# maplant/mgf

Hardware: AMD Instinct MI355X
Metric: contact_constraint_iters_per_sec (higher is better)
Workload: dtype f32

## Files before the change

mgf_amd/csrc/host_boundary.inc:

```

extern "C" mgf_status mgf_constraints_new(mgf_world* w, const mgf_body_ref* refs_a, const mgf_body_ref* refs_b, const mgf_manifold* manifolds,
                                          int64_t n, float dt, mgf_constraint* out, int64_t cap, int64_t* count) {
  if (!w || n < 0 || (n && (!refs_a || !refs_b || !manifolds))) return fail(MGF_ERR_INVALID, "bad argument");
  MGF_TRY(ctx_bind(w->ctx));
  MGF_TRY(perm_host(w));
  const uint32_t* so = w->permuted ? w->h_slot_of.data() : nullptr;
  std::vector<ManifoldRow> rows;
  std::vector<uint2> names;
  for (int64_t i = 0; i < n; ++i) {
    const mgf_body_ref& ra = refs_a[i];
    const mgf_body_ref& rb = refs_b[i];
    const mgf_manifold& m = manifolds[i];
    if (ra.tag != 0) return fail(MGF_ERR_STATIC_REF, "obj_a must be RigidBodyRef::Dynamic");
    if (ra.index >= w->n_owned) return fail(MGF_ERR_INVALID, "obj_a out of range");
    if (rb.tag == 0 && rb.index >= w->n_owned) return fail(MGF_ERR_INVALID, "obj_b out of range");
    if (rb.tag != 0 && rb.tag != 1) return fail(MGF_ERR_INVALID, "obj_b: unknown RigidBodyRef tag");
    if (rb.tag == 0 && rb.index == ra.index) return fail(MGF_ERR_INVALID, "a constraint needs two different bodies");
    if (m.n_contacts < 0 || m.n_contacts > MGF_MANIFOLD_CAP) return fail(MGF_ERR_INVALID, "manifold: n_contacts out of range");
    for (int32_t k = 0; k < m.n_contacts; ++k) {
      ManifoldRow r;
      r.a = ra.index; r.b = rb.tag == 0 ? rb.index : kNone;
      names.push_back(make_uint2(r.a, r.b));
      if (so) { r.a = so[r.a]; if (r.b != kNone) r.b = so[r.b]; }
      r.cb[0] = rb.center.x; r.cb[1] = rb.center.y; r.cb[2] = rb.center.z; r.fric_b = rb.friction;
// ... 53 lines not shown
  if (count) *count = (int64_t)s->cons.size();
  if (!out) return MGF_OK;
  if ((int64_t)s->cons.size() > cap) return fail(MGF_ERR_CAPACITY, "constraint buffer too small");
  if (!s->cons.empty()) memcpy(out, s->cons.data(), s->cons.size() * sizeof(mgf_constraint));
  return MGF_OK;
}
extern "C" mgf_status mgf_solver_solve(mgf_solver* s, mgf_world* w, int32_t iters, mgf_step_stats* stats) {
  if (!s || !w) return fail(MGF_ERR_INVALID, "NULL argument");
  if (iters < 0) return fail(MGF_ERR_INVALID, "iters must be >= 0");
  w->n = w->n_owned;
  mgf_status st = mgf_world_set_constraints(w, s->cons.data(), (int64_t)s->cons.size());
  if (st == MGF_OK) st = mgf_world_solve(w, iters, stats);
  if (st == MGF_OK && !s->cons.empty()) st = mgf_world_read_constraints(w, s->cons.data(), (int64_t)s->cons.size(), nullptr);
  return st;
}

template <class T>
static mgf_status clone_buf(mgf_ctx* ctx, DBuf<T>& dst, const DBuf<T>& src, size_t count) {
  if (count == 0 || !src.p) return MGF_OK;
  MGF_TRY(dst.ensure(count, ctx->stream));
  MGF_HIP_TRY(hipMemcpyAsync(dst.p, src.p, count * sizeof(T), hipMemcpyDeviceToDevice, ctx->stream));
  return MGF_OK;
}
extern "C" mgf_status mgf_world_clone(mgf_world* src, mgf_world** out) {
  if (!src || !out) return fail(MGF_ERR_INVALID, "NULL argument");
  *out = nullptr;
  mgf_world* w = nullptr;
  MGF_TRY(mgf_world_new(src->ctx, &src->params, &w));
  std::unique_ptr<mgf_world, void (*)(mgf_world*)> guard(w, mgf_world_free);
  mgf_ctx* ctx = src->ctx;
  const size_t n = src->n_owned;
  MGF_TRY(clone_buf(ctx, w->x, src->x, n)); MGF_TRY(clone_buf(ctx, w->q, src->q, n)); MGF_TRY(clone_buf(ctx, w->srec, src->srec, 4 * n));
  MGF_TRY(clone_buf(ctx, w->sp0, src->sp0, n)); MGF_TRY(clone_buf(ctx, w->sp1, src->sp1, n)); MGF_TRY(clone_buf(ctx, w->ctor, src->ctor, n));
  MGF_TRY(clone_buf(ctx, w->imb, src->imb, 3 * n)); MGF_TRY(clone_buf(ctx, w->delta, src->delta, n)); MGF_TRY(clone_buf(ctx, w->einfo, src->einfo, n));
  MGF_TRY(clone_buf(ctx, w->col0, src->col0, n)); MGF_TRY(clone_buf(ctx, w->col1, src->col1, n)); MGF_TRY(clone_buf(ctx, w->tb_c, src->tb_c, n));
  MGF_TRY(clone_buf(ctx, w->tb_r, src->tb_r, n)); MGF_TRY(clone_buf(ctx, w->fb_c, src->fb_c, n)); MGF_TRY(clone_buf(ctx, w->fb_r, src->fb_r, n));
  if (src->has_compound) {
    MGF_TRY(clone_buf(ctx, w->pcount, src->pcount, n));
    MGF_TRY(clone_buf(ctx, w->lp0, src->lp0, kMaxParts * n)); MGF_TRY(clone_buf(ctx, w->lp1, src->lp1, kMaxParts * n));
    MGF_TRY(clone_buf(ctx, w->wp0, src->wp0, kMaxParts * n)); MGF_TRY(clone_buf(ctx, w->wp1, src->wp1, kMaxParts * n));
    MGF_TRY(clone_buf(ctx, w->xl0, src->xl0, src->x_used)); MGF_TRY(clone_buf(ctx, w->xl1, src->xl1, src->x_used));
    MGF_TRY(clone_buf(ctx, w->xw0, src->xw0, src->x_used)); MGF_TRY(clone_buf(ctx, w->xw1, src->xw1, src->x_used));
    w->x_used = src->x_used;
  }
  if (src->permuted) {
    MGF_TRY(clone_buf(ctx, w->ext_of, src->ext_of, n)); MGF_TRY(clone_buf(ctx, w->slot_of, src->slot_of, n));
    w->permuted = true;
  }
  w->opt_resort_every = src->opt_resort_every; w->ticks_since_resort = src->ticks_since_resort;
  MGF_HIP_TRY(hipStreamSynchronize(ctx->stream));
  w->n = w->n_owned = src->n_owned;
  w->has_sphere = src->has_sphere; w->has_capsule = src->has_capsule; w->has_compound = src->has_compound; w->max_parts = src->max_parts;
  w->stats.n_bodies = w->n_owned;
  if (src->terrain) MGF_TRY(mgf_world_set_terrain(w, src->terrain.get()));
  for (const auto& ob : src->obstacles) MGF_TRY(mgf_world_add_obstacle(w, ob.get()));
  w->opt_constraint_order = src->opt_constraint_order; w->demo_tree = src->demo_tree; w->demo_leaf = src->demo_leaf;
  w->opt_flow6_poll_prio = src->opt_flow6_poll_prio; w->opt_flow6_slot_blocks = src->opt_flow6_slot_blocks; w->opt_resort_partition = src->opt_resort_partition; w->opt_part_cell_x8 = src->opt_part_cell_x8;
  w->opt_flow6_poll_k = src->opt_flow6_poll_k; w->opt_flow6_spec = src->opt_flow6_spec; w->opt_flow6_spec_wl = src->opt_flow6_spec_wl; w->opt_flow6_test_cap = src->opt_flow6_test_cap; w->opt_flow_trace = src->opt_flow_trace; w->opt_debug_bvh = src->opt_debug_bvh;
  w->opt_flow6_fcap = src->opt_flow6_fcap; w->opt_flow6_const_lds = src->opt_flow6_const_lds; w->opt_flow6_nimp_lds = src->opt_flow6_nimp_lds; w->opt_flow6_rec_lds = src->opt_flow6_rec_lds; w->opt_flow6_slot_margin = src->opt_flow6_slot_margin; w->opt_flow6_quad = src->opt_flow6_quad; w->opt_flow6_quad_max = src->opt_flow6_quad_max; w->opt_flow6_foreign_lds = src->opt_flow6_foreign_lds; w->opt_flow6_poll_waves = src->opt_flow6_poll_waves;
  w->opt_solver_mode = src->opt_solver_mode; w->opt_two_pass = src->opt_two_pass; w->opt_broadphase_tree = src->opt_broadphase_tree;
  w->opt_terrain_tree = src->opt_terrain_tree; w->opt_no_fused_narrowphase = src->opt_no_fused_narrowphase;
  w->opt_no_fused_scene_bounds = src->opt_no_fused_scene_bounds; w->opt_no_fused_terrain_rows = src->opt_no_fused_terrain_rows;
  w->opt_pair_brick = src->opt_pair_brick; w->opt_body_pack = src->opt_body_pack; w->opt_grid_min_frac_pct = src->opt_grid_min_frac_pct;
  w->grid_occupancy = src->grid_occupancy;
  w->opt_cell_fill = src->opt_cell_fill; w->opt_cell_fill_set = src->opt_cell_fill_set; w->opt_pipeline = src->opt_pipeline; w->opt_spin_wait = src->opt_spin_wait; w->opt_readback_kernel = src->opt_readback_kernel;
  w->opt_stream_ordered = src->opt_stream_ordered; w->opt_flow_blocks_per_cu = src->opt_flow_blocks_per_cu; w->opt_flow_sleep = src->opt_flow_sleep;
  w->opt_flow5_slow_x2 = src->opt_flow5_slow_x2; w->opt_flow5_poller = src->opt_flow5_poller; w->opt_flow5_block = src->opt_flow5_block;
  w->opt_flow5_test_cap = src->opt_flow5_test_cap; w->opt_time_solver_kernels = src->opt_time_solver_kernels; w->opt_phase_timing = src->opt_phase_timing;
  w->row_cap_t = src->row_cap_t; w->rev_cap = src->rev_cap; w->pair_brick_off = src->pair_brick_off; w->pair_brick_backoff = src->pair_brick_backoff; w->terrain_grid_off = src->terrain_grid_off; w->grid_too_wide = src->grid_too_wide;
  w->cap_t = src->cap_t; w->cap_p = src->cap_p; w->cap_c = src->cap_c; w->flow5_last_max = src->flow5_last_max;
  w->f6_fail_slots = src->f6_fail_slots; w->f6_fail_foreign = src->f6_fail_foreign; w->f6_fail_C = src->f6_fail_C; w->prev_C = src->prev_C;
  w->f6_last_slots = src->f6_last_slots; w->f6_last_foreign = src->f6_last_foreign; w->f6_last_msgs = src->f6_last_msgs;
  w->f6_last_block_msgs = src->f6_last_block_msgs; w->f6_prep_iters = src->f6_prep_iters;
  w->opt_merged_lists = src->opt_merged_lists; w->opt_fused_contacts = src->opt_fused_contacts; w->opt_front_rows = src->opt_front_rows; w->opt_front_rows_check = src->opt_front_rows_check; w->opt_side_stream = src->opt_side_stream; w->opt_wide_list = src->opt_wide_list; w->wide_engaged = src->wide_engaged; w->wide_hold = src->wide_hold;
  for (int k = 0; k < 3; ++k) { w->wide_ref[k] = src->wide_ref[k]; w->wide_limit[k] = src->wide_limit[k]; w->shape_rmax[k] = src->shape_rmax[k]; } w->front_rows_off = src->front_rows_off; w->opt_flow_max_blocks = src->opt_flow_max_blocks; w->opt_cells_in_integrate = src->opt_cells_in_integrate; w->opt_resort_every = src->opt_resort_every;
  for (int k = 0; k < 3; ++k) { w->h_scene_ext[k] = src->h_scene_ext[k]; w->h_scene_rmax[k] = src->h_scene_rmax[k]; }
  *out = guard.release();
  return MGF_OK;
}
```

mgf_amd/csrc/host_tick.inc:

```
enum TerrainPlan { kTerrainNone, kTerrainRows, kTerrainGrid };
static TerrainPlan terrain_plan(const mgf_world* w, bool two_pass) {
  if (two_pass || !w->terrain || w->terrain->m.tree.empty() || !w->n_owned) return kTerrainNone;
  return (w->terrain->grid.ready && !w->terrain_grid_off && !w->opt_terrain_tree && w->obstacles.empty()) ? kTerrainGrid : kTerrainRows;
}
static mgf_status world_integrate(mgf_world* w, float dt, bool complete, bool integrate, bool with_bounds, bool with_terrain_rows = false) {
  mgf_ctx* ctx = w->ctx;
  w->invalidate_tick_caches();
  if (w->n_owned == 0) return MGF_OK;
  SceneBounds* sb = with_bounds ? w->sb.p : nullptr;
  const uint32_t* guard = with_bounds ? w->scalars.p + 14 : nullptr;
  int* sb_part = (with_terrain_rows && integrate && with_bounds && !w->opt_no_fused_scene_bounds) ? w->sb_part.p : nullptr;
  w->bounds_cover = sb_part ? w->n_owned : 0u;
  MGF_TRY(w->bpk.ensure(4 * (size_t)std::max(w->n, w->n_owned), ctx->stream));
  w->pack_cover = integrate ? w->n_owned : 0u;
  CellSort cs;
  memset(&cs, 0, sizeof(cs));
  if (sb_part && w->plan.zero_launched && w->plan.n == w->n_owned && w->sbg_valid && w->opt_cells_in_integrate) {
    cs.grid = w->sb_grid.p; cs.shift = kMortonBits - 2 * (int)w->plan.levels; cs.min_frac = (float)w->opt_grid_min_frac_pct * 0.01f;
    cs.cell_of = w->cell_of.p; cs.rank = w->cell_rank.p; cs.cell_cnt = w->cell_cnt.p;
    w->cells_cover = w->n_owned; w->cells_levels = w->plan.levels;
  }
  WideSpec wd;
  memset(&wd, 0, sizeof(wd));
  w->wide_tick_on = false;
  if (sb_part && integrate && w->opt_wide_list && w->wide_engaged && w->wide_limit[0] > 0.0f) {
    MGF_TRY(w->wide_list.ensure(2 * (size_t)kWideCap, ctx->stream));
    for (int k = 0; k < 3; ++k) wd.limit[k] = w->wide_limit[k];
    wd.list = w->wide_list.p; wd.count = &w->sb.p->pad; wd.ext = w->ext_ptr();
    w->wide_tick_on = true;
  }
  if (with_terrain_rows && integrate && terrain_plan(w, w->opt_two_pass != 0) == kTerrainRows && !w->opt_no_fused_terrain_rows) {
    MGF_TRY(w->rows_t.ensure((size_t)w->n_owned * w->row_cap_t, ctx->stream));
    MGF_TRY(w->t_cnt.ensure((size_t)w->n_owned + 1, ctx->stream));
    MGF_TRY(w->near_list.ensure(3 * (size_t)w->n_owned, ctx->stream)); MGF_TRY(w->cs_sums.ensure(3 * kCsSumStride, ctx->stream));
    TerrainRowsTail tail{w->terrain->dev(w->d_err()), w->row_cap_t, w->rows_t.p, w->t_cnt.p, w->d_err() + 1, w->opt_fused_contacts ? w->near_list.p : nullptr, w->cs_sums.p + 2 * kCsSumStride};
    k_integrate<<<nblk(w->n_owned), kBlock, 0, ctx->stream>>>(w->bodies(), w->n_owned, dt, w->params.fat_margin, complete ? 1 : 0, 1, sb, guard, tail, sb_part, cs, wd);
    w->terrain_rows_done = true;
  } else {
    k_integrate<<<nblk(w->n_owned), kBlock, 0, ctx->stream>>>(w->bodies(), w->n_owned, dt, w->params.fat_margin, complete ? 1 : 0, integrate ? 1 : 0,
                                                        sb, guard, NoTail(), sb_part, cs, wd);
  }
  LAUNCH_CHECK();
  return MGF_OK;
}
extern "C" mgf_status mgf_world_complete_motion(mgf_world* w) {
  if (!w) return fail(MGF_ERR_INVALID, "world is NULL");
  MGF_TRY(ctx_bind(w->ctx));
  MGF_TRY(world_integrate(w, 0.0f, true, false, false));
  MGF_HIP_TRY(hipStreamSynchronize(w->ctx->stream));
  return MGF_OK;
}
extern "C" mgf_status mgf_world_integrate(mgf_world* w, float dt) {
  if (!w) return fail(MGF_ERR_INVALID, "world is NULL");
  MGF_TRY(ctx_bind(w->ctx));
  MGF_TRY(world_integrate(w, dt, false, true, false));
  MGF_HIP_TRY(hipStreamSynchronize(w->ctx->stream));
  return MGF_OK;
}

static mgf_status launch_pairs(mgf_world* w, int ka, int kb, const uint32_t* work, const uint32_t* m_ptr, uint32_t cap, bool pack_ok) {
  if (cap == 0) return MGF_OK;
  hipStream_t s = w->ctx->stream;
  Bodies B = w->bodies();
  if (!pack_ok) B.bpk = nullptr;
  unsigned g = nblk(cap);
  if (ka == 0 && kb == 0) k_narrow_pairs<0, 0><<<g, kBlock, 0, s>>>(B, work, m_ptr, w->p_owner.p, w->p_cand.p, w->p_nc.p, w->p_out.p);
  else if (ka == 0 && kb == 1) k_narrow_pairs<0, 1><<<g, kBlock, 0, s>>>(B, work, m_ptr, w->p_owner.p, w->p_cand.p, w->p_nc.p, w->p_out.p);
  else if (ka == 1 && kb == 0) k_narrow_pairs<1, 0><<<g, kBlock, 0, s>>>(B, work, m_ptr, w->p_owner.p, w->p_cand.p, w->p_nc.p, w->p_out.p);
  else k_narrow_pairs<1, 1><<<g, kBlock, 0, s>>>(B, work, m_ptr, w->p_owner.p, w->p_cand.p, w->p_nc.p, w->p_out.p);
  LAUNCH_CHECK();
  return MGF_OK;
}
static mgf_status launch_terrain(mgf_world* w, int ka, const TerrainDev& M, const uint32_t* work, const uint32_t* m_ptr, uint32_t cap, bool pack_ok) {
  if (cap == 0) return MGF_OK;
  hipStream_t s = w->ctx->stream;
  Bodies B = w->bodies();
  if (!pack_ok) B.bpk = nullptr;
  unsigned g = nblk(cap);
  if (ka == 0) k_narrow_terrain<0><<<g, kBlock, 0, s>>>(B, M, work, m_ptr, w->t_owner.p, w->t_cand.p, w->t_nc.p, w->t_out.p);
  else k_narrow_terrain<1><<<g, kBlock, 0, s>>>(B, M, work, m_ptr, w->t_owner.p, w->t_cand.p, w->t_nc.p, w->t_out.p);
  LAUNCH_CHECK();
  return MGF_OK;
}

static mgf_status links_ensure(mgf_world* w, uint32_t cap_c, bool zero = false) {
  hipStream_t s = w->ctx->stream;
  uint32_t n = w->n;
  MGF_TRY(w->c_ab.ensure(std::max(cap_c, 1u), s)); MGF_TRY(w->c_succ.ensure(std::max(cap_c, 1u), s)); MGF_TRY(w->c_pred.ensure(2 * (size_t)std::max(cap_c, 1u), s));
  MGF_TRY(w->deg.ensure(n + 1, s)); MGF_TRY(w->adj_off.ensure(n + 1, s)); MGF_TRY(w->adj_fill.ensure(n + 1, s));
  MGF_TRY(w->adj_list.ensure(2 * (size_t)std::max(cap_c, 1u), s));
  if (zero) {
    MGF_HIP_TRY(hipMemsetAsync(w->deg.p, 0, (n + 1) * 4, s));
    MGF_HIP_TRY(hipMemsetAsync(w->adj_fill.p, 0, (n + 1) * 4, s));
  }
  return MGF_OK;
}
static mgf_status build_dag(mgf_world* w, uint32_t cap_c) {
  mgf_ctx* ctx = w->ctx;
  hipStream_t s = ctx->stream;
  uint32_t n = w->n;
  w->depth = 0;
  if (cap_c == 0) return MGF_OK;
  if (cap_c >= kSuccId) return fail(MGF_ERR_CAPACITY, "too many constraints");
  MGF_TRY(prim_exclusive_scan_u32(ctx, w->deg.p, w->adj_off.p, (size_t)n + 1));
  k_adj_fill<<<nblk(cap_c), kBlock, 0, s>>>(w->c_ab.p, &w->sc.p->C, w->adj_off.p, w->adj_fill.p, w->adj_list.p);
  LAUNCH_CHECK();
  k_chain<<<nblk(n), kBlock, 0, s>>>(n, w->links(), w->adj_off.p, w->adj_list.p);
  LAUNCH_CHECK();
  return MGF_OK;
}
// ... 170 lines not shown
      bool ok = false;
      MGF_TRY(flow6_plan(w, cap_c, w->f6_prep_iters ? w->f6_prep_iters : 10u, &ok));
      if (ok) { flow6_zero_entries(w, cap_c, z, 8); w->flow6_zeroed = true; }
    }
    if (solver_follows && w->opt_solver_mode == 5) {
      bool ok = false;
      MGF_TRY(flow5_plan(w, cap_c, &ok));
      if (ok) { flow5_zero_entries(w, cap_c, z, 8); w->flow5_zeroed = true; }
    }
    if (early) {
      k_tick_clear<<<256, kBlock, 0, s>>>(z, w->sb.p, w->d_err(), w->scalars.p + 14, &w->sc.p->fail, speculative ? 1 : 0, w->sb_part.p);
      w->plan.zero_launched = true;
    } else {
      if (bounds_done) { z.sb = w->sb.p; z.sb_part = w->sb_part.p; }
      k_zero_many<<<256, kBlock, 0, s>>>(z);
      w->plan.zero_launched = false;
    }
    LAUNCH_CHECK();
  }
  return MGF_OK;
}
static mgf_status collide_enqueue(mgf_world* w, float dt, bool solver_follows = false) {
  mgf_ctx* ctx = w->ctx;
  hipStream_t s = ctx->stream;
  const uint32_t n = w->n;
  StepCounts* sc = w->sc.p;
  if (n == 0) { MGF_HIP_TRY(hipMemsetAsync(sc, 0, sizeof(StepCounts), s)); return MGF_OK; }
  Bodies B = w->bodies();
  const float min_frac = (float)w->opt_grid_min_frac_pct * 0.01f;
  const bool cleared = w->plan.zero_launched && w->plan.n == n && w->plan.cap_c == w->cap_c && w->plan.solver_follows == solver_follows && w->cap_p != 0;
  w->plan.zero_launched = false;
  const bool bounds_done = w->bounds_cover == n && n > 0;
  const bool rows_done = w->terrain_rows_done;
  const bool pack_ok = w->pack_cover == n && n > 0 && w->opt_body_pack;
  if (!cleared) MGF_TRY(collide_prepare(w, solver_follows, false, false));
  const uint32_t cap_t = w->cap_t, cap_p = w->cap_p, cap_c = w->cap_c;
  const uint32_t levels = w->plan.levels, cells = w->plan.cells, nblocks = cells / kBlock;
  if (!pack_ok) B.bpk = nullptr;
  const bool cells_done = cleared && bounds_done && w->cells_cover == n && w->cells_levels == w->plan.levels;
  w->invalidate_tick_caches();
  const bool fold_in_morton = cleared && bounds_done;
  if (!bounds_done) {
    k_scene_bounds<<<std::min<unsigned>(nblk(n), 64u), kBlock, 0, s>>>(w->fb_c.p, w->fb_r.p, n, w->sb.p);
    LAUNCH_CHECK();
  }
  if (!cells_done) {
    k_morton_count<<<nblk(n), kBlock, 0, s>>>(w->fb_c.p, n, w->sb.p, kMortonBits - 2 * (int)levels, w->cell_of.p, w->cell_rank.p, w->cell_cnt.p, min_frac, make_uint3(0, 0, 0),
                                              fold_in_morton ? w->sb_part.p : nullptr, w->sb.p);
    LAUNCH_CHECK();
  }
  const SceneBounds* grid_box_of = cells_done ? w->sb_grid.p : nullptr;
  MGF_TRY(tick_scan(w, 0, w->cell_cnt.p, w->cell_lo.p, nullptr, nullptr, (size_t)cells + 1, nullptr, nullptr, cells_done ? w->sb_part.p : nullptr));
  Lbvh T;
  T.nodes = w->lnodes.p; T.leaves = w->leaves.p; T.sidx = w->sidx.p; T.cell_lo = w->cell_lo.p;
  T.n = n; T.levels = levels; T.err = w->d_err();
  T.dbg = nullptr;
  T.ext = w->ext_ptr();
  const bool two_pass = (w->opt_two_pass != 0 || w->tick_two_pass) && !w->demo_rows_ready;
  const bool use_grid = !two_pass && !w->opt_broadphase_tree && !w->grid_too_wide;
  const bool demo = w->demo_rows_ready;
  const bool fused = use_grid && !w->has_capsule && !w->has_compound && !w->opt_no_fused_narrowphase && !demo;
  T.lcol = nullptr; T.ltb = nullptr;
  if (fused) { MGF_TRY(w->lcol.ensure(2 * (size_t)n, s)); T.lcol = w->lcol.p; }
  const bool wide_now = w->wide_tick_on && bounds_done && use_grid && !two_pass && !demo;
  const float3 wlim = wide_now ? make_float3(w->wide_limit[0], w->wide_limit[1], w->wide_limit[2]) : make_float3(0.0f, 0.0f, 0.0f);
  const bool brick = use_grid && !demo && w->opt_pair_brick && w->pair_brick_off == 0 && !wide_now;
  if (w->pair_brick_off) --w->pair_brick_off;
  w->ts->brick = brick;
  if (use_grid && !demo) { MGF_TRY(w->ltb.ensure(2 * (size_t)n, s)); T.ltb = w->ltb.p; }
  if (brick) {
    if (!w->pair_brick_attr) {
// ... 43 lines not shown
    }
    MGF_TRY(w->near_ids.ensure(w->n_owned, s)); MGF_TRY(w->tpos.ensure(n + 1, s));
    const FaceGrid FG = w->terrain->face_grid();
    k_near_list<<<nblk(w->n_owned), kBlock, 0, ts>>>(w->tb_c.p, w->tb_r.p, w->n_owned, M, FG.sb, 1e-3f, w->near_ids.p, w->cs_sums.p + 2 * kCsSumStride, w->scalars.p + 14);
    LAUNCH_CHECK();
    TerrainNear A;
    A.M = M; A.G = FG; A.near_ids = w->near_ids.p; A.near_cnt = w->cs_sums.p + 2 * kCsSumStride; A.face_of_rank = w->terrain->grid.face_of_rank.p;
    const uint32_t region_cap = slot_space / kTnRegions;
    A.pad_abs = 1e-3f; A.cap_t = cap_t; A.cnt = w->front_cnt.p; A.region_cap = region_cap; A.slot_body = w->t_owner.p; A.slot_rank = w->t_cand.p; A.tpos = w->tpos.p; A.t_cnt = w->t_cnt.p;
    A.overflow = w->d_err() + 1; A.too_wide = w->d_err() + 5; A.guard = w->scalars.p + 14;
    A.check = w->opt_front_rows_check ? 1u : 0u;
#ifndef MGF_TN_LANES
#define MGF_TN_LANES 16
#endif
    constexpr int kTnLanes = MGF_TN_LANES;
    const unsigned tgb = 8u * std::max(1u, std::min((unsigned)((w->n_owned + (kBlock / kTnLanes) - 1) / (kBlock / kTnLanes) + 7u) / 8u, 256u));
    k_terrain_near<kTnLanes><<<tgb, kBlock, 0, ts>>>(B, A);
    LAUNCH_CHECK();
    TerrainTests X;
    X.M = M; X.face_of_rank = w->terrain->grid.face_of_rank.p; X.slot_body = w->t_owner.p; X.slot_rank = w->t_cand.p; X.cnt = w->front_cnt.p; X.region_cap = region_cap;
    X.t_out = w->t_out.p; X.tcn = w->tcn.p; X.sum_ct = w->cs_sums.p + kCsSumStride; X.flag = w->d_err() + 8; X.overflow = w->d_err() + 1;
    k_terrain_tests<<<nblk((size_t)region_cap * kTnRegions), kBlock, 0, ts>>>(B, X);
    LAUNCH_CHECK();
    if (forked) MGF_HIP_TRY(hipEventRecord(w->ts->ev_join, ctx->aux));
  }
  if (tc_job) {
    const uint32_t t_stride0 = w->has_compound ? 2u * (w->max_parts > 2u ? (uint32_t)kMaxParts : 2u) : 2u;
    MGF_TRY(w->t_out.ensure((size_t)t_stride0 * cap_t, s)); MGF_TRY(w->tpos.ensure(n + 1, s));
    TerrainContacts A;
    A.M = M; A.near_list = w->near_list.p; A.near_cnt = w->cs_sums.p + 2 * kCsSumStride;
    A.n_faces = (uint32_t)(w->terrain->faces.size() / 3); A.n_verts = (uint32_t)w->terrain->verts.size(); A.cap_row_t = w->row_cap_t; A.cap_t = cap_t;
    A.rows_t = w->rows_t.p; A.sums = w->cs_sums.p; A.t_out = w->t_out.p; A.tcn = w->tcn.p; A.tpos = w->tpos.p; A.guard = w->scalars.p + 14;
    A.check = (front_rows && w->opt_front_rows_check) ? 1u : 0u; A.flag = w->d_err() + 8;
    A.col1 = w->col1.p; A.pcount = w->has_compound ? w->pcount.p : nullptr; A.wp0 = w->wp0.p; A.wp1 = w->wp1.p;
    const unsigned tg = std::max(1u, std::min(nblk((size_t)w->n_owned * kTcLanes / 8 + 1), 256u));
    if (front_rows) {
      hipStream_t ts = s;
      if (w->opt_side_stream && !w->opt_phase_timing) {
        if (!ctx->aux) {
          int lo = 0, hi = 0;
          MGF_HIP_TRY(hipDeviceGetStreamPriorityRange(&lo, &hi));
          MGF_HIP_TRY(hipStreamCreateWithPriority(&ctx->aux, hipStreamNonBlocking, w->opt_side_stream >= 2 ? lo : hi));
        }
        if (!w->ts->ev_fork) { MGF_HIP_TRY(hipEventCreateWithFlags(&w->ts->ev_fork, hipEventDisableTiming)); MGF_HIP_TRY(hipEventCreateWithFlags(&w->ts->ev_join, hipEventDisableTiming)); }
        MGF_HIP_TRY(hipEventRecord(w->ts->ev_fork, s));
        MGF_HIP_TRY(hipStreamWaitEvent(ctx->aux, w->ts->ev_fork, 0));
        ts = ctx->aux; forked = true;
      }
      if (w->has_compound) k_terrain_contacts<2><<<tg, kBlock, 0, ts>>>(A);
      else k_terrain_contacts<1><<<tg, kBlock, 0, ts>>>(A);
      LAUNCH_CHECK();
      if (forked) MGF_HIP_TRY(hipEventRecord(w->ts->ev_join, ts));
      k_scatter_leaves<<<nblk(n), kBlock, 0, s>>>(T, w->fb_c.p, w->fb_r.p, w->cell_of.p, w->cell_rank.p, w->brank.p, w->col0.p, w->delta.p, w->tb_c.p, w->tb_r.p, w->sb.p, 1e-3f, min_frac, grid_box_of, wlim, w->n_owned);
    } else if (w->opt_fused_contacts >= 2) {
      k_terrain_contacts<0><<<tg, kBlock, 0, s>>>(A);
      LAUNCH_CHECK();
      k_scatter_leaves<<<nblk(n), kBlock, 0, s>>>(T, w->fb_c.p, w->fb_r.p, w->cell_of.p, w->cell_rank.p, w->brank.p, w->col0.p, w->delta.p, w->tb_c.p, w->tb_r.p, w->sb.p, 1e-3f, min_frac, grid_box_of, wlim, w->n_owned);
    } else {
      k_scatter_leaves_tc<0><<<nblk(n) + tg, kBlock, 0, s>>>(T, w->fb_c.p, w->fb_r.p, w->cell_of.p, w->cell_rank.p, w->brank.p, w->col0.p, w->delta.p, w->tb_c.p, w->tb_r.p, w->sb.p, 1e-3f, min_frac, A, tg, grid_box_of, wlim, w->n_owned);
    }
  } else {
    k_scatter_leaves<<<nblk(n), kBlock, 0, s>>>(T, w->fb_c.p, w->fb_r.p, w->cell_of.p, w->cell_rank.p, w->brank.p, w->col0.p, w->delta.p, w->tb_c.p, w->tb_r.p, w->sb.p, 1e-3f, min_frac, grid_box_of, wlim, w->n_owned);
  }
  LAUNCH_CHECK();
  w->sidx_valid = n == w->n_owned;
  if (!use_grid) {
    k_lbvh_low<<<nblocks, kBlock, 0, s>>>(T, w->sub_lo.p, w->sub_hi.p);
    LAUNCH_CHECK();
    if (levels > 4) { k_lbvh_top<<<1, 1024, 0, s>>>(T, w->sub_lo.p, w->sub_hi.p, w->sub2_lo.p, w->sub2_hi.p); LAUNCH_CHECK(); }
  }
  MGF_TRY(phase_mark(w, 1, s));
  MGF_TRY(w->t_cand.ensure(cap_t, s)); MGF_TRY(w->t_owner.ensure(cap_t, s));
  MGF_TRY(w->p_cand.ensure(cap_p, s)); MGF_TRY(w->p_owner.ensure(cap_p, s));
  MGF_TRY(w->t_nc.ensure(cap_t, s)); MGF_TRY(w->p_nc.ensure(cap_p, s));
  MGF_TRY(w->t_pre.ensure(cap_t, s)); MGF_TRY(w->p_pre.ensure(cap_p, s));
  const uint32_t MP = w->max_parts > 2u ? (uint32_t)kMaxParts : 2u;
  const bool big = w->max_parts > (uint32_t)kMaxParts;
  const uint32_t t_stride = w->has_compound ? 2u * (big ? w->max_parts : MP) : 2u, p_stride = w->has_compound ? MP * MP : 1u;
  static_assert(kBigKeep == (uint32_t)(kMaxParts * kMaxParts), "k_narrow_pairs_big writes k_narrow_pairs_parts<kMaxParts>'s records");
  MGF_TRY(w->t_out.ensure((size_t)t_stride * cap_t, s)); MGF_TRY(w->p_out.ensure((size_t)p_stride * cap_p, s));
  if (!two_pass) {
    MGF_TRY(w->rows.ensure((size_t)n * kRowCap, s));
    MGF_TRY(w->rows_t.ensure((size_t)n * w->row_cap_t, s, rows_done, (size_t)w->n_owned * w->row_cap_t));
    if (front_rows && terrain_any && terrain_grid) {
    } else if (M.n_nodes && w->n_owned && !rows_done) {
      if (terrain_grid) {
        const uint32_t per_block = kCoopBlock / kCoopLanes;
        const uint32_t tg = 8 * (((w->n_owned + per_block - 1) / per_block + 7) / 8);
        k_terrain_grid<<<tg, kCoopBlock, 0, s>>>(B, w->n_owned, nullptr, M, w->terrain->face_grid(), 1e-3f, w->row_cap_t, w->rows_t.p, w->t_cnt.p,
                                                 w->d_err() + 1, w->d_err() + 5);
      } else {
        k_terrain_rows<<<nblk(w->n_owned), kBlock, 0, s>>>(B, w->n_owned, M, w->row_cap_t, w->rows_t.p, w->t_cnt.p, w->d_err() + 1);
      }
      LAUNCH_CHECK();
    }
// ... 78 lines not shown
  } else if (two_pass) {
    k_candidates<true><<<8 * xcd_blocks_per(n), kBlock, 0, s>>>(B, n, w->n_owned, T, M, 1e-3f, nullptr, nullptr, w->t_off.p, w->p_off.p, w->t_cand.p, w->t_owner.p,
                                                  w->p_cand.p, w->p_owner.p, sc);
    if (n_obs && w->n_owned) {
      LAUNCH_CHECK();
      k_obstacle_candidates<true><<<nblk(w->n_owned), kBlock, 0, s>>>(B, w->n_owned, w->d_obs.p, n_obs, w->t_cnt.p, w->t_off.p, w->t_cand.p, w->t_owner.p, sc);
    }
  } else {
    k_rows_to_csr<<<nblk(n), kBlock, 0, s>>>(sc, n, w->row_cap_t, terrain_grid ? w->terrain->grid.face_of_rank.p : nullptr, w->rows_t.p, w->rows.p, w->t_off.p, w->p_off.p, w->t_cand.p, w->t_owner.p, w->p_cand.p, w->p_owner.p);
  }
  LAUNCH_CHECK();
  MGF_TRY(phase_mark(w, 2, s));
  bool mixed = w->has_sphere && w->has_capsule;
  if (lists_merged || front_rows) {
  } else if (w->has_compound) {
    if (cap_p && big) {
      k_narrow_pairs_big<<<std::min(std::max(cap_p / 4u, 1u), 4096u), kBlock, 0, s>>>(B, &sc->Mp, w->p_owner.p, w->p_cand.p, w->p_nc.p, w->p_out.p, w->scalars.p + 24);
      LAUNCH_CHECK();
    } else if (cap_p) {
      if (MP == 2u) k_narrow_pairs_parts<2><<<nblk(cap_p), kBlock, 0, s>>>(B, &sc->Mp, w->p_owner.p, w->p_cand.p, w->p_nc.p, w->p_out.p);
      else k_narrow_pairs_parts<kMaxParts><<<nblk(cap_p), kBlock, 0, s>>>(B, &sc->Mp, w->p_owner.p, w->p_cand.p, w->p_nc.p, w->p_out.p);
      LAUNCH_CHECK();
    }
    if ((M.n_nodes || n_obs) && cap_t && big) {
      k_narrow_terrain_big<<<std::min(std::max(cap_t / 4u, 1u), 4096u), kBlock, 0, s>>>(B, M, &sc->Mt, w->t_owner.p, w->t_cand.p, w->t_nc.p, w->t_out.p, t_stride);
      LAUNCH_CHECK();
    } else if ((M.n_nodes || n_obs) && cap_t) {
      if (MP == 2u) k_narrow_terrain_parts<2><<<nblk(cap_t), kBlock, 0, s>>>(B, M, &sc->Mt, w->t_owner.p, w->t_cand.p, w->t_nc.p, w->t_out.p);
      else k_narrow_terrain_parts<kMaxParts><<<nblk(cap_t), kBlock, 0, s>>>(B, M, &sc->Mt, w->t_owner.p, w->t_cand.p, w->t_nc.p, w->t_out.p);
      LAUNCH_CHECK();
    }
  } else if (!mixed) {
    int k = w->has_capsule ? 1 : 0;
    if (!fused) MGF_TRY(launch_pairs(w, k, k, nullptr, &sc->Mp, cap_p, pack_ok));
    if (M.n_nodes || n_obs) MGF_TRY(launch_terrain(w, k, M, nullptr, &sc->Mt, cap_t, pack_ok));
  } else {
    MGF_TRY(w->work_lists.ensure(4 * (size_t)cap_p + 2 * (size_t)cap_t, s));
    uint32_t* lists_p = w->work_lists.p;
    uint32_t* lists_t = w->work_lists.p + 4 * (size_t)cap_p;
    k_bin_pairs<<<nblk(cap_p), kBlock, 0, s>>>(B, &sc->Mp, cap_p, w->p_owner.p, w->p_cand.p, lists_p, sc->bins);
    LAUNCH_CHECK();
    for (int ty = 0; ty < 4; ++ty) MGF_TRY(launch_pairs(w, ty >> 1, ty & 1, lists_p + (size_t)ty * cap_p, &sc->bins[ty], cap_p, pack_ok));
    if (M.n_nodes || n_obs) {
      k_bin_terrain<<<nblk(cap_t), kBlock, 0, s>>>(B, &sc->Mt, cap_t, w->t_owner.p, lists_t, sc->bins + 4);
      LAUNCH_CHECK();
      for (int ty = 0; ty < 2; ++ty) MGF_TRY(launch_terrain(w, ty, M, lists_t + (size_t)ty * cap_t, &sc->bins[4 + ty], cap_t, pack_ok));
    }
  }
  if (n_obs && cap_t) {
    k_narrow_obstacles<<<nblk(cap_t), kBlock, 0, s>>>(B, w->d_obs.p, &sc->Mt, w->t_owner.p, w->t_cand.p, w->t_nc.p, w->t_out.p, t_stride);
    LAUNCH_CHECK();
  }
  MGF_TRY(phase_mark(w, 3, s));
  MGF_TRY(w->cnt.ensure(n + 1, s)); MGF_TRY(w->base.ensure(n + 1, s)); MGF_TRY(w->tcn.ensure(n + 1, s));
  if (!contacts_fused && !front_rows) {
  if (!lists_merged) {
    k_count_contacts<<<nblk(n), kBlock, 0, s>>>(sc, n, w->t_off.p, w->p_off.p, w->t_nc.p, fused ? nullptr : w->p_nc.p, w->p_cand.p, w->t_pre.p, w->p_pre.p, w->cnt.p,
                                                demo ? 1 : 0, w->tcn.p, w->ext_ptr());
    LAUNCH_CHECK();
  }
  {
    ScanEpilogue E;
    memset(&E, 0, sizeof(E));
    E.kind = 2; E.cap_a = cap_c; E.sc = sc;
    MGF_TRY(tick_scan(w, 2, w->cnt.p, w->base.p, nullptr, nullptr, (size_t)n + 1, &E));
  }
  TerrainSetup TS;
  memset(&TS, 0, sizeof(TS));
  if (M.n_nodes || n_obs) {
    TS.M = M; TS.t_owner = w->t_owner.p; TS.t_nc = w->t_nc.p; TS.t_pre = w->t_pre.p; TS.t_in = w->t_out.p; TS.in_stride = t_stride; TS.blocks = nblk(cap_t);
    if (n_obs) { TS.t_cand = w->t_cand.p; TS.obs_center = w->d_obs_center.p; }
  }
  if (fused) k_setup_pairs<true><<<TS.blocks + nblk(cap_p), kBlock, 0, s>>>(B, sc, w->p_owner.p, w->p_cand.p, nullptr, w->p_pre.p, nullptr, w->base.p, dt,
                                                                            w->params.baumgarte, w->params.penetration_slop, w->cons_nat.p, w->c_ab.p, w->degb.p, w->rev.p,
                                                                            w->rev_cap, w->d_err() + 7, p_stride, w->d_err() + 8, TS, w->ext_ptr());
  else k_setup_pairs<false><<<TS.blocks + nblk(cap_p), kBlock, 0, s>>>(B, sc, w->p_owner.p, w->p_cand.p, w->p_nc.p, w->p_pre.p, w->p_out.p, w->base.p, dt,
                                                                       w->params.baumgarte, w->params.penetration_slop, w->cons_nat.p, w->c_ab.p, w->degb.p, w->rev.p,
                                                                       w->rev_cap, w->d_err() + 7, p_stride, w->d_err() + 8, TS, w->ext_ptr());
  LAUNCH_CHECK();
// ... 214 lines not shown
```

mgf_amd/csrc/host_tiles.inc:

```
template <class Batch, class Tile>
static mgf_status tile_batches(hipStream_t s, void (*kern)(Batch), const Tile* tiles, const uint32_t* blocks, int L) {
  for (int i0 = 0; i0 < L; i0 += kTileBatch) {
    Batch A;
    memset(&A, 0, sizeof(A));
    const int cnt = std::min(kTileBatch, L - i0);
    uint32_t mx = 0;
    for (int k = 0; k < cnt; ++k) { A.t[k] = tiles[i0 + k]; mx = std::max(mx, blocks[i0 + k]); }
    if (!mx) continue;
    kern<<<dim3(mx, (unsigned)cnt), kBlock, 0, s>>>(A);
    LAUNCH_CHECK();
  }
  return MGF_OK;
}
static mgf_status select_describe(mgf_world* w, float x_left, float x_right, float x_lo, float x_hi, uint32_t* ids_l, uint32_t* ids_r, uint32_t* ids_m, SelTile* S) {
  const uint32_t n = w->n_owned, nb = nblk(n);
  MGF_TRY(w->sel_blk.ensure(4 * (size_t)nb + 4, w->ctx->stream));
  S->fb_c = w->fb_c.p; S->fb_r = w->fb_r.p; S->x = w->x.p; S->n = n;
  S->x_left = x_left; S->x_right = x_right; S->x_lo = x_lo; S->x_hi = x_hi;
  S->blk = w->sel_blk.p; S->tot = w->sel_blk.p + 4 * (size_t)nb; S->tot_host = nullptr;
  S->ids_l = ids_l; S->ids_r = ids_r; S->ids_m = ids_m;
  return MGF_OK;
}
static mgf_status select_counts(hipStream_t s, const SelTile* sel, int L) {
  std::vector<uint32_t> blocks((size_t)L);
// ... 46 lines not shown
  MGF_TRY(grow_keep(w, w->pcount, 1, need));
  MGF_TRY(grow_keep(w, w->lp0, kMaxParts, need)); MGF_TRY(grow_keep(w, w->lp1, kMaxParts, need));
  MGF_TRY(grow_keep(w, w->wp0, kMaxParts, need)); MGF_TRY(grow_keep(w, w->wp1, kMaxParts, need));
  return MGF_OK;
}
static mgf_status raise_parts_for_records(mgf_world* w, const float* rec, int64_t m, uint32_t stride_floats, uint32_t at) {
  if (m <= 0 || !rec) return MGF_OK;
  MGF_TRY(w->mig_cnt.ensure(2, w->ctx->stream));
  MGF_HIP_TRY(hipMemsetAsync(w->mig_cnt.p, 0, 8, w->ctx->stream));
  k_record_max_parts<<<nblk(m), kBlock, 0, w->ctx->stream>>>(rec, (uint32_t)m, stride_floats, at, w->mig_cnt.p);
  LAUNCH_CHECK();
  uint32_t pc = 0;
  MGF_TRY(d2h(w->ctx, &pc, w->mig_cnt.p, 1));
  if (pc > (uint32_t)kTileParts) return fail(MGF_ERR_INVALID, "a record claims more parts than a tile record carries");
  if (pc > 2u && w->max_parts <= 2u) return mgf_world_set_option(w, "body_kinds", 12);
  if (pc > 0u && !w->has_compound) return mgf_world_set_option(w, "body_kinds", 4);
  return MGF_OK;
}
static mgf_status world_import_ghosts2(mgf_world* w, const float* src, int64_t n_ghost, const float* src2, int64_t n_first);
extern "C" mgf_status mgf_world_import_ghosts(mgf_world* w, const float* src, int64_t n_ghost) {
  if (w && src && n_ghost > 0 && !w->opt_stream_ordered) { MGF_TRY(ctx_bind(w->ctx)); MGF_TRY(raise_parts_for_records(w, src, n_ghost, (uint32_t)kGhostFloats, 36u)); }
  return world_import_ghosts2(w, src, n_ghost, nullptr, n_ghost);
}
static mgf_status world_import_ghosts_prepare(mgf_world* w, const float* src, int64_t n_ghost, const float* src2, int64_t n_first, ImpTile* I) {
  memset(I, 0, sizeof(*I));
  if (w) w->sbg_valid = false;
  if (!w || (n_ghost && !src && !src2) || n_ghost < 0 || n_first < 0 || (n_first < n_ghost && !src2) || (n_first > 0 && n_ghost > 0 && !src)) return fail(MGF_ERR_INVALID, "bad argument");
  MGF_TRY(ctx_bind(w->ctx));
  MGF_TRY(world_identity(w));
  size_t need = (size_t)w->n_owned + (size_t)n_ghost;
  if (need > 0x7FFFFFF0ull) return fail(MGF_ERR_INVALID, "too many bodies");
  MGF_TRY(grow_keep(w, w->x, 1, need)); MGF_TRY(grow_keep(w, w->q, 1, need)); MGF_TRY(grow_keep(w, w->srec, 4, need));
  MGF_TRY(grow_keep(w, w->sp0, 1, need)); MGF_TRY(grow_keep(w, w->sp1, 1, need)); MGF_TRY(grow_keep(w, w->ctor, 1, need));
  MGF_TRY(grow_keep(w, w->imb, 3, need)); MGF_TRY(grow_keep(w, w->delta, 1, need)); MGF_TRY(grow_keep(w, w->einfo, 1, need));
  MGF_TRY(grow_keep(w, w->col0, 1, need)); MGF_TRY(grow_keep(w, w->col1, 1, need)); MGF_TRY(grow_keep(w, w->tb_c, 1, need));
  MGF_TRY(grow_keep(w, w->tb_r, 1, need)); MGF_TRY(grow_keep(w, w->fb_c, 1, need)); MGF_TRY(grow_keep(w, w->fb_r, 1, need));
  MGF_TRY(grow_parts(w, need));
  MGF_TRY(grow_keep(w, w->bpk, 4, need));
  w->pack_cover = (w->pack_cover >= w->n_owned && w->n_owned > 0) ? (uint32_t)need : 0u;
  if (n_ghost > 0) {
    const bool join = w->bounds_cover == w->n_owned && w->n == w->n_owned && w->n_owned > 0;
    I->B = w->bodies(); I->n_owned = w->n_owned; I->m = (uint32_t)n_ghost; I->m1 = (uint32_t)std::min<int64_t>(n_first, n_ghost);
    I->fat_margin = w->params.fat_margin; I->in = src; I->in2 = src2; I->sb_part = join ? w->sb_part.p : nullptr;
    I->rec1 = I->rec2 = (uint32_t)kGhostFloats;
    w->bounds_cover = join ? (uint32_t)need : 0u;
  } else if (w->n != w->n_owned) {
    w->bounds_cover = 0;
  }
  w->n = (uint32_t)need;
  w->constraints_ready = false;
  return MGF_OK;
}
static mgf_status world_import_ghosts2(mgf_world* w, const float* src, int64_t n_ghost, const float* src2, int64_t n_first) {
  ImpTile I;
  MGF_TRY(world_import_ghosts_prepare(w, src, n_ghost, src2, n_first, &I));
  const uint32_t blocks = nblk(I.m);
  MGF_TRY((tile_batches<ImpBatch, ImpTile>(w->ctx->stream, k_import_ghosts, &I, &blocks, 1)));
  return sync_unless_ordered(w);
}
extern "C" mgf_status mgf_world_select_tile(mgf_world* w, float x_left, float x_right, float x_lo, float x_hi, uint32_t* ids_left,
                                            uint32_t* ids_right, uint32_t* ids_migrants, int64_t cap, int64_t* counts) {
  if (!w || !counts) return fail(MGF_ERR_INVALID, "NULL argument");
  MGF_TRY(ctx_bind(w->ctx));
  MGF_TRY(world_identity(w));
  mgf_ctx* ctx = w->ctx;
  hipStream_t s = ctx->stream;
  counts[0] = counts[1] = counts[2] = counts[3] = 0;
  if (w->n_owned == 0) return MGF_OK;
  SelTile S;
  MGF_TRY(select_describe(w, x_left, x_right, x_lo, x_hi, ids_left, ids_right, ids_migrants, &S));
  MGF_TRY(select_counts(s, &S, 1));
// ... 59 lines not shown
  if (!trusted) {
    uint32_t* pin = static_cast<uint32_t*>(ctx->pinned);
    MGF_HIP_TRY(hipMemcpyAsync(pin, w->mig_cnt.p, 4, hipMemcpyDeviceToHost, s));
    MGF_HIP_TRY(hipStreamSynchronize(s));
    if (pin[0]) return fail(MGF_ERR_INVALID, "remove_bodies: an id is out of range or listed twice");
  }
  const uint32_t n_new = n - (uint32_t)n_ids;
  if (n_new) {
    k_compact_put<<<dim3(nblk(n_new), row_words), kBlock, 0, s>>>(w->bodies(), n, n_new, w->bscan_l.p, w->mig_tmp.p);
    LAUNCH_CHECK();
  }
  w->n_owned = w->n = n_new;
  w->stats.n_bodies = n_new;
  w->sidx_valid = false;
  w->demo_tree.clear(); w->demo_leaf.clear();
  return sync_unless_ordered(w);
}
extern "C" mgf_status mgf_world_remove_bodies(mgf_world* w, const uint32_t* ids, int64_t n_ids) { return remove_bodies_impl(w, ids, n_ids, false); }
static mgf_status import_migrants_impl(mgf_world* w, const float* src, int64_t n_in, uint32_t kinds_hint, const float* src2 = nullptr, int64_t n_first = -1) {
  if (n_first < 0 || n_first > n_in) n_first = n_in;
  if (!w || n_in < 0 || (n_first > 0 && !src) || (n_first < n_in && (!src2 || !kinds_hint))) return fail(MGF_ERR_INVALID, "bad argument");
  w->invalidate_tick_caches();
  MGF_TRY(ctx_bind(w->ctx));
  MGF_TRY(world_identity(w));
  w->n = w->n_owned;
  w->constraints_ready = false;
  if (n_in == 0) return MGF_OK;
  size_t need = (size_t)w->n_owned + (size_t)n_in;
  if (need > 0x7FFFFFF0ull) return fail(MGF_ERR_INVALID, "too many bodies");
  w->sbg_valid = false; w->ptrs_out = false;
  if (!kinds_hint) MGF_TRY(raise_parts_for_records(w, src, n_in, 4u * (uint32_t)kMigrantWords, 4u * 20u));
  MGF_TRY(grow_keep(w, w->x, 1, need)); MGF_TRY(grow_keep(w, w->q, 1, need)); MGF_TRY(grow_keep(w, w->srec, 4, need));
  MGF_TRY(grow_keep(w, w->sp0, 1, need)); MGF_TRY(grow_keep(w, w->sp1, 1, need)); MGF_TRY(grow_keep(w, w->ctor, 1, need));
  MGF_TRY(grow_keep(w, w->imb, 3, need)); MGF_TRY(grow_keep(w, w->delta, 1, need)); MGF_TRY(grow_keep(w, w->einfo, 1, need));
  MGF_TRY(grow_keep(w, w->col0, 1, need)); MGF_TRY(grow_keep(w, w->col1, 1, need)); MGF_TRY(grow_keep(w, w->tb_c, 1, need));
  MGF_TRY(grow_keep(w, w->tb_r, 1, need)); MGF_TRY(grow_keep(w, w->fb_c, 1, need)); MGF_TRY(grow_keep(w, w->fb_r, 1, need));
  MGF_TRY(grow_parts(w, need));
  k_import_migrants<<<nblk((size_t)n_in * kMigrantWords), kBlock, 0, w->ctx->stream>>>(w->bodies(), w->n_owned, (uint32_t)n_in,
                                                                                      reinterpret_cast<const float4*>(src), kTileParts,
                                                                                      reinterpret_cast<const float4*>(src2), (uint32_t)n_first);
  LAUNCH_CHECK();
  w->n_owned = w->n = (uint32_t)need;
  w->stats.n_bodies = w->n_owned;
  w->sidx_valid = false;
  if (kinds_hint) {
    if (kinds_hint & 1u) w->has_sphere = true;
    if (kinds_hint & 2u) w->has_capsule = true;
    return MGF_OK;
  }
  MGF_TRY(w->mig_cnt.ensure(2, w->ctx->stream));
  MGF_HIP_TRY(hipMemsetAsync(w->mig_cnt.p, 0, 8, w->ctx->stream));
  k_kind_mask<<<nblk(n_in), kBlock, 0, w->ctx->stream>>>(w->col1.p, w->has_compound ? w->pcount.p : nullptr, w->n_owned - (uint32_t)n_in, (uint32_t)n_in, w->mig_cnt.p);
  LAUNCH_CHECK();
  uint32_t mask = 0;
  MGF_TRY(d2h(w->ctx, &mask, w->mig_cnt.p, 1));
  if (mask & 1) w->has_sphere = true;
  if (mask & 2) w->has_capsule = true;
  return MGF_OK;
}
extern "C" mgf_status mgf_world_import_migrants(mgf_world* w, const float* src, int64_t n_in) { return import_migrants_impl(w, src, n_in, 0u); }
extern "C" mgf_status mgf_world_set_tags(mgf_world* w, const uint32_t* tags, int64_t n) {
  if (!w || (n && !tags)) return fail(MGF_ERR_INVALID, "NULL argument");
  if ((uint64_t)n != (uint64_t)w->n_owned) return fail(MGF_ERR_INVALID, "one tag per owned body");
  MGF_TRY(ctx_bind(w->ctx));
  if (n == 0) return MGF_OK;
  MGF_TRY(w->bflag_l.ensure((size_t)n + 1, w->ctx->stream));
  if (w->permuted) {
    MGF_TRY(perm_host(w));
    std::vector<uint32_t> t((size_t)n);
    for (size_t i = 0; i < (size_t)n; ++i) t[w->h_slot_of[i]] = tags[i];
    MGF_TRY(h2d(w->ctx, w->bflag_l.p, t.data(), (size_t)n));
  } else {
    MGF_TRY(h2d(w->ctx, w->bflag_l.p, tags, (size_t)n));
  }
  k_tags_set<<<nblk(n), kBlock, 0, w->ctx->stream>>>(w->ctor.p, w->bflag_l.p, (uint32_t)n);
  LAUNCH_CHECK();
  MGF_HIP_TRY(hipStreamSynchronize(w->ctx->stream));
  return MGF_OK;
}
extern "C" mgf_status mgf_world_read_tags(mgf_world* w, uint32_t* tags, int64_t cap) {
  if (!w || (cap && !tags)) return fail(MGF_ERR_INVALID, "NULL argument");
  if ((uint64_t)cap < (uint64_t)w->n_owned) return fail(MGF_ERR_CAPACITY, "tag buffer too small");
  MGF_TRY(ctx_bind(w->ctx));
  const uint32_t n = w->n_owned;
  if (n == 0) return MGF_OK;
// ... 43 lines not shown
```

mgf_amd/csrc/host_world.inc:

```
struct mgf_world {
  mgf_ctx* ctx = nullptr;
  mgf_params params;
  uint32_t n = 0;
  uint32_t n_owned = 0;
  bool has_sphere = false, has_capsule = false;
  bool has_compound = false;
  uint32_t max_parts = 0;
  DBuf<uint32_t> pcount;
  DBuf<float4> xl0, xl1, xw0, xw1;
  uint32_t x_used = 0;
  DBuf<float4> lp0, lp1, wp0, wp1;
  DBuf<uint32_t> bflag_l, bscan_l;
  DBuf<uint32_t> sel_blk;
  DBuf<uint32_t> mig_cnt;
  DBuf<float4> mig_tmp;
  DBuf<float> state_pack;
  void* state_pin = nullptr; size_t state_pin_bytes = 0;
  DBuf<float4> x, q, srec, sp0, sp1, ctor, imb, delta, einfo, col0, col1, tb_c, tb_r, fb_c, fb_r;
  DBuf<float4> bpk;
  DBuf<uint32_t> ext_of, ext_new, slot_of;
  DBuf<float4> perm_tmp;
  bool permuted = false;
  bool sidx_valid = false;
  int64_t opt_resort_every = -1;
  uint64_t ticks_since_resort = 0, n_resorts = 0;
  std::vector<uint32_t> h_ext_of, h_slot_of;
  bool h_perm_valid = false;
  const uint32_t* ext_ptr() const { return permuted ? ext_of.p : nullptr; }
  DBuf<uint32_t> part_keys[2], part_vals[2];
  int64_t opt_part_cell_x8 = 4;
  int64_t opt_resort_partition = 1;
  float h_scene_ext[3] = {0, 0, 0};
  float h_scene_rmax[3] = {0, 0, 0};
  bool list_generic = false;
  DBuf<uint32_t> f6_cslot, f6_clist;
  DBuf<uint32_t> iota;
  size_t iota_n = 0;
  int64_t opt_flow6_slot_blocks = 1;
  DBuf<uint32_t> cnt_e, base_e, canon;
  bool canon_ready = false;
  std::unique_ptr<mgf_mesh> terrain;
  std::vector<std::unique_ptr<mgf_compound>> obstacles;
  DBuf<CompoundDev> d_obs;
  DBuf<float4> d_obs_center;
  DBuf<uint32_t> cell_of, cell_rank, sidx;
  DBuf<QNode> lnodes;
  DBuf<LeafRec> leaves;
  DBuf<float4> ltb;
  DBuf<float4> lcol;
  int64_t opt_no_fused_narrowphase = 0;
  int64_t opt_grid_min_frac_pct = 50;
  int64_t opt_merged_lists = 1;
  int64_t opt_cells_in_integrate = 1;
  int64_t opt_front_rows = 1;
  int64_t opt_wide_list = 1;
  bool wide_engaged = false, wide_tick_on = false;
  float wide_ref[3] = {0, 0, 0}, wide_limit[3] = {0, 0, 0};
  float shape_rmax[3] = {0, 0, 0};
  uint32_t wide_hold = 0, wide_last = 0;
  uint64_t n_wide_ticks = 0, n_wide_overflows = 0;
  uint64_t n_path_ticks[4] = {0, 0, 0, 0};
  DBuf<float4> wide_list;
  DBuf<float4> q_bc, q_br;
  DBuf<uint32_t> q_cnt, q_start, q_items, q_large, q_misc, q_off, q_vals;
  DBuf<ParticleIn> q_parts; DBuf<int32_t> q_ign, q_hits; DBuf<float> q_boxes;
  DBuf<MovingIn> q_casts;
  uint32_t q_last_large = 0, q_last_cells = 0;
  float q_last_build_ms = 0.0f, q_last_run_ms = 0.0f;
  int64_t opt_side_stream = 1;
  int64_t opt_front_rows_check = 0;
  bool front_rows_off = false;
  int64_t opt_fused_contacts = 1;
  int64_t opt_body_pack = 1;
  int64_t opt_pair_brick = 1;
  uint64_t pair_brick_slow = 0;
  uint32_t pair_brick_off = 0;
  uint32_t pair_brick_backoff = 256;
  bool pair_brick_attr = false;
  DBuf<float4> sub_lo, sub_hi, sub2_lo, sub2_hi;
  DBuf<uint32_t> cell_lo, cell_cnt;
  DBuf<uint32_t> t_cnt, p_cnt, t_off, p_off, t_cand, t_owner, p_cand, p_owner, rows, rows_t;
  int64_t opt_solver_mode = 6;
  DBuf<uint32_t> flow_arr, flow_arr5;
  DBuf<uint64_t> flow_trace;
  DBuf<uint32_t> brank, f5_shared, f5_gcnt, f5_lslot, f5_wg_cnt;
  DBuf<F5Row> f5_table;
  bool flow5_zeroed = false;
  bool f6_fail_known = false;
  uint32_t f6_fail_host = 0;
  bool f6_standby = false;
  uint32_t f6_edges_block = 0;
  bool links_ready = false;
  bool flow5_ok = false, flow5_prepped = false;
  uint32_t f5_nb = 0, f5_nblocks = 0;
  DBuf<uint4> f6_binfo;
  DBuf<uint32_t> f6_bref, f6_fcnt, f6_fbody, f6_nslots, f6_in_key, f6_in_cnt, f6_out_key, f6_out_val, f6_chan_prefix;
  DBuf<uint8_t> f6_cflags, f6_skipwb;
  DBuf<F6Row> f6_table;
  DBuf<uint4> f6_mbox;
  DBuf<unsigned long long> f6_tails;
  uint32_t f6_mbox_cap = 0;
  uint32_t f6_epoch = 0;
  uint32_t f6_fcap = 512, f6_slot_cap = 0, f6_rows = 0;
  uint32_t f6_last_slots = 0, f6_last_foreign = 0;
  uint32_t f6_fail_slots = 0, f6_fail_foreign = 0, f6_fail_C = 0, prev_C = 0;
  uint64_t n_flow6_skipped = 0;
// ... 102 lines not shown
  View<SceneBounds> sb;
  uint32_t Mt = 0, Mp = 0, C = 0, Ct = 0, depth = 0, last_launches = 0, lvl_cap = 0;
  size_t order_cap_iters = 0;
  bool constraints_ready = false;
  float last_dt = 0.0f;
  float last_rmax_x = 0.0f;
  float grid_occupancy = 1.0f;
  int64_t opt_time_solver_kernels = 0;
  int64_t opt_phase_timing = 0;
  struct TickSlot {
    hipEvent_t ev[8] = {};
    uint32_t ev_set = 0;
    std::vector<hipEvent_t> kev;
    size_t kev_used = 0;
    bool brick = false;
    bool fused = false;
    bool front_rows = false;
    bool contacts_fused = false;
    bool cells_early = false;
    hipEvent_t ev_fork = nullptr, ev_join = nullptr;
    uint32_t* pin = nullptr;
    uint32_t* pin_dev = nullptr;
    uint32_t seq = 0;
  };
  static constexpr uint32_t kPinWords = 4096, kPinSeqWord = 4095;
  void* pin_block = nullptr;
  TickSlot slots[2];
  TickSlot* ts = &slots[0];
  mgf_step_stats stats;

  Bodies bodies() {
    Bodies B;
    B.x = x.p; B.q = q.p; B.srec = srec.p; B.sp0 = sp0.p; B.sp1 = sp1.p; B.ctor = ctor.p; B.imb = imb.p; B.bpk = bpk.p; B.delta = delta.p;
    B.einfo = einfo.p; B.col0 = col0.p; B.col1 = col1.p; B.tb_c = tb_c.p; B.tb_r = tb_r.p; B.fb_c = fb_c.p; B.fb_r = fb_r.p;
    B.pcount = has_compound ? pcount.p : nullptr; B.lp0 = lp0.p; B.lp1 = lp1.p; B.wp0 = wp0.p; B.wp1 = wp1.p;
    B.xl0 = xl0.p; B.xl1 = xl1.p; B.xw0 = xw0.p; B.xw1 = xw1.p;
    return B;
  }
  uint32_t* d_cnt() { return scalars.p; }
  uint32_t* d_err() { return scalars.p + 3; }
  uint32_t flow5_narrow_cap() const { return f5_narrow_cap(f5_nb); }
  Flow5 flow5() {
    Flow5 F;
    F.sidx = sidx.p; F.brank = brank.p; F.shared = reinterpret_cast<uint8_t*>(f5_shared.p);
    F.gcnt = f5_gcnt.p; F.arr5 = flow_arr5.p; F.lslot = f5_lslot.p; F.wg_cnt = f5_wg_cnt.p;
    F.table = f5_table.p;
    F.fail = d_err() + 4; F.max_block = d_err() + 6;
    F.cap_fast = flow5_wide ? kF5MaxFast : flow5_narrow_cap(); F.cap_slow = flow5_wide ? kF5MaxSlow : flow5_narrow_cap();
    F.cap_all = flow5_wide ? kF5MaxCons : flow5_narrow_cap();
    if (opt_flow5_test_cap > 0) F.cap_all = std::min<uint32_t>(F.cap_all, (uint32_t)opt_flow5_test_cap);
    F.slow_x2 = (uint32_t)opt_flow5_slow_x2;
    F.poller = opt_flow5_poller < 0 ? (flow5_wide ? 0u : 1u) : (uint32_t)opt_flow5_poller;
    F.nb = f5_nb; F.nblocks = f5_nblocks; F.n = n;
    return F;
  }
  ConsLinks links() { ConsLinks K; K.ab = c_ab.p; K.succ = c_succ.p; K.pred = c_pred.p; return K; }
  Frontier frontier() { Frontier F; F.order = order.p; F.lvl_off = lvl_off.p; F.cnt = d_cnt(); return F; }
};
static mgf_status phase_mark(mgf_world* w, int k, hipStream_t s) {
  if (!w->opt_phase_timing) return MGF_OK;
  MGF_HIP_TRY(hipEventRecord(w->ts->ev[k], s));
  w->ts->ev_set |= 1u << k;
  return MGF_OK;
}
static mgf_status phase_ms(mgf_world* w, int a, int b, float* ms) {
  *ms = 0.0f;
  if (!w->opt_phase_timing || (w->ts->ev_set & (1u << a)) == 0u || (w->ts->ev_set & (1u << b)) == 0u) return MGF_OK;
// ... 75 lines not shown
  if (!strcmp(key, "flow6_nimp_lds")) { w->opt_flow6_nimp_lds = value; return MGF_OK; }
  if (!strcmp(key, "flow6_rec_lds")) { w->opt_flow6_rec_lds = value; return MGF_OK; }
  if (!strcmp(key, "flow6_slot_margin")) { if (value < 0 || value > 1024) return fail(MGF_ERR_INVALID, "flow6_slot_margin: 0..1024"); w->opt_flow6_slot_margin = value; return MGF_OK; }
  if (!strcmp(key, "flow6_quad")) { w->opt_flow6_quad = value; return MGF_OK; }
  if (!strcmp(key, "flow6_quad_max")) { if (value < -1 || value > 1000000) return fail(MGF_ERR_INVALID, "flow6_quad_max out of range"); w->opt_flow6_quad_max = value; return MGF_OK; }
  if (!strcmp(key, "flow6_foreign_lds")) { w->opt_flow6_foreign_lds = value; return MGF_OK; }
  if (!strcmp(key, "flow6_test_cap")) { w->opt_flow6_test_cap = value; return MGF_OK; }
  if (!strcmp(key, "flow6_poll_prio")) { if (value < 0 || value > 3) return fail(MGF_ERR_INVALID, "flow6_poll_prio: 0..3"); w->opt_flow6_poll_prio = value; return MGF_OK; }
  if (!strcmp(key, "flow6_spec_wl")) { if (value < -1 || value > 8) return fail(MGF_ERR_INVALID, "flow6_spec_wl: -1..8"); w->opt_flow6_spec_wl = value; return MGF_OK; }
  if (!strcmp(key, "flow6_spec")) { if (value < 0 || value > 8) return fail(MGF_ERR_INVALID, "flow6_spec: 0 (by the launch), 1..8"); w->opt_flow6_spec = value; return MGF_OK; }
  if (!strcmp(key, "flow6_poll_waves")) { if (value < 0 || value > 4) return fail(MGF_ERR_INVALID, "flow6_poll_waves out of range"); w->opt_flow6_poll_waves = value; return MGF_OK; }
  if (!strcmp(key, "flow6_poll_k")) { if (value < 1 || value > 4) return fail(MGF_ERR_INVALID, "flow6_poll_k out of range"); w->opt_flow6_poll_k = value; return MGF_OK; }
  if (!strcmp(key, "flow_blocks_per_cu")) { w->opt_flow_blocks_per_cu = value; w->flow_grid = 0; w->flowk_grid = 0; return MGF_OK; }
  if (!strcmp(key, "flow_sleep")) { w->opt_flow_sleep = value; return MGF_OK; }
  if (!strcmp(key, "flow5_poller")) { w->opt_flow5_poller = value < 0 ? -1 : (value ? 1 : 0); return MGF_OK; }
  if (!strcmp(key, "flow5_slow_x2")) { if (value < 1 || value > 16) return fail(MGF_ERR_INVALID, "flow5_slow_x2 out of range"); w->opt_flow5_slow_x2 = value; return MGF_OK; }
  if (!strcmp(key, "flow5_test_cap")) { w->opt_flow5_test_cap = value; return MGF_OK; }
  if (!strcmp(key, "flow5_block")) { w->opt_flow5_block = value; w->flow5_prepped = false; return MGF_OK; }
  if (!strcmp(key, "no_fused_narrowphase")) { w->opt_no_fused_narrowphase = value; return MGF_OK; }
  if (!strcmp(key, "pair_brick")) { w->opt_pair_brick = value; return MGF_OK; }
  if (!strcmp(key, "merged_lists")) { w->opt_merged_lists = value; return MGF_OK; }
  if (!strcmp(key, "fused_contacts")) { w->opt_fused_contacts = value; return MGF_OK; }
  if (!strcmp(key, "front_rows")) { w->opt_front_rows = value; return MGF_OK; }
  if (!strcmp(key, "side_stream")) { w->opt_side_stream = value; return MGF_OK; }
  if (!strcmp(key, "wide_list")) { w->opt_wide_list = value; if (!value) w->wide_engaged = false; return MGF_OK; }
  if (!strcmp(key, "front_rows_check")) { w->opt_front_rows_check = value; return MGF_OK; }
  if (!strcmp(key, "cells_in_integrate")) { w->opt_cells_in_integrate = value; return MGF_OK; }
  if (!strcmp(key, "flow_spin_limit")) { if (value < 0 || value > (4 << 20)) return fail(MGF_ERR_INVALID, "flow_spin_limit: 0 .. 4194304"); w->opt_flow_spin_limit = value; return MGF_OK; }
  if (!strcmp(key, "flow_max_blocks")) {
    if (value < 0 || value > 4096) return fail(MGF_ERR_INVALID, "flow_max_blocks: 0 (one workgroup per CU) .. 4096");
    w->opt_flow_max_blocks = value; w->flow_grid = 0; w->flowk_grid = 0; w->flow5_prepped = false; w->flow6_prepped = false;
    return MGF_OK;
  }
  if (!strcmp(key, "body_pack")) { w->opt_body_pack = value; return MGF_OK; }
  if (!strcmp(key, "grid_min_frac_pct")) { if (value < 0 || value > 100) return fail(MGF_ERR_INVALID, "grid_min_frac_pct: 0..100"); w->opt_grid_min_frac_pct = value; return MGF_OK; }
  if (!strcmp(key, "cell_fill")) { if (value < 1 || value > 1024) return fail(MGF_ERR_INVALID, "cell_fill out of range"); w->opt_cell_fill = value; w->opt_cell_fill_set = true; return MGF_OK; }
  if (!strcmp(key, "no_fused_scene_bounds")) { w->opt_no_fused_scene_bounds = value; return MGF_OK; }
  if (!strcmp(key, "no_fused_terrain_rows")) { w->opt_no_fused_terrain_rows = value; return MGF_OK; }
  if (!strcmp(key, "part_cell_x8")) { if (value < 0 || value > 64) return fail(MGF_ERR_INVALID, "part_cell_x8: 0..64"); w->opt_part_cell_x8 = value; return MGF_OK; }
  if (!strcmp(key, "resort_partition")) { w->opt_resort_partition = value; return MGF_OK; }
  if (!strcmp(key, "flow6_slot_blocks")) { w->opt_flow6_slot_blocks = value; return MGF_OK; }
  if (!strcmp(key, "resort_every")) {
    if (value < -1 || value > 1000000) return fail(MGF_ERR_INVALID, "resort_every out of range");
    w->opt_resort_every = value;
    if (value == 0) MGF_TRY(world_identity(w));
    return MGF_OK;
  }
  if (!strcmp(key, "pipeline")) { w->opt_pipeline = value; return MGF_OK; }
  if (!strcmp(key, "spin_wait")) { w->opt_spin_wait = value; return MGF_OK; }
  if (!strcmp(key, "readback_kernel")) { w->opt_readback_kernel = value != 0; return MGF_OK; }
  if (!strcmp(key, "stream_ordered")) { w->opt_stream_ordered = value; return MGF_OK; }
  if (!strcmp(key, "body_kinds")) {
    if (value & 1) w->has_sphere = true;
    if (value & 2) w->has_capsule = true;
    if ((value & 12) == 12) w->max_parts = std::max(w->max_parts, (uint32_t)kMaxParts);
    else if (value & 4) w->max_parts = std::max(w->max_parts, 2u);
    if ((value & 4) && !w->has_compound) {
      MGF_TRY(ctx_bind(w->ctx));
      const size_t o = w->n_owned;
      std::vector<uint32_t> pz(o, 0u);
      std::vector<float4> fz(kMaxParts * o, make_float4(0, 0, 0, 0));
      MGF_TRY(append(w->ctx, w->pcount, 0, pz));
      MGF_TRY(append(w->ctx, w->lp0, 0, fz)); MGF_TRY(append(w->ctx, w->lp1, 0, fz));
      MGF_TRY(append(w->ctx, w->wp0, 0, fz)); MGF_TRY(append(w->ctx, w->wp1, 0, fz));
      w->has_compound = true;
    }
    return MGF_OK;
// ... 199 lines not shown
      float best_len = 0.0f;
      for (int k = 0; k < 3; ++k) {
        const float len = (hi[k] - lo[k]) / (float)(1u << bits[k]);
        if (bits[k] < 10u && len * 0.5f >= 2.0f * rmax[k] && len * 0.5f > 0.0f && len > best_len) { best = k; best_len = len; }
      }
      if (best < 0) break;
      ++bits[best];
    }
    G.bits[0] = bits[0]; G.bits[1] = bits[1]; G.bits[2] = bits[2];
  }
  const uint32_t cells = 1u << (G.bits[0] + G.bits[1] + G.bits[2]);
  G.levels = levels; G.n_faces = (uint32_t)nf;
  MGF_TRY(G.fb_c.ensure(nf, s)); MGF_TRY(G.fb_r.ensure(nf, s)); MGF_TRY(G.cell_of.ensure(nf, s)); MGF_TRY(G.cell_rank.ensure(nf, s));
  MGF_TRY(G.cell_cnt.ensure((size_t)cells + 1, s)); MGF_TRY(G.cell_lo.ensure((size_t)cells + 1, s)); MGF_TRY(G.sidx.ensure(nf, s));
  MGF_TRY(G.brank.ensure(nf, s)); MGF_TRY(G.leaves.ensure(nf, s)); MGF_TRY(G.sb.ensure(1, s));
  MGF_TRY(G.rank_of_face.ensure(nf, s)); MGF_TRY(G.face_of_rank.ensure(nf, s)); MGF_TRY(G.leaf_of_face.ensure(nf, s));
  MGF_TRY(G.parent.ensure(std::max<size_t>(parent.size(), 1), s));
  MGF_TRY(h2d(ctx, G.fb_c.p, bc.data(), nf)); MGF_TRY(h2d(ctx, G.fb_r.p, br.data(), nf));
  MGF_TRY(h2d(ctx, G.rank_of_face.p, rank_of.data(), nf)); MGF_TRY(h2d(ctx, G.face_of_rank.p, face_of.data(), nf));
  MGF_TRY(h2d(ctx, G.leaf_of_face.p, leaf_of.data(), nf)); MGF_TRY(h2d(ctx, G.parent.p, parent.data(), parent.size()));
  MGF_HIP_TRY(hipMemsetAsync(G.cell_cnt.p, 0, ((size_t)cells + 1) * 4, s));
  SceneBounds sb0;
  for (int k = 0; k < 3; ++k) { sb0.lo[k] = 0x7FFFFFFF; sb0.hi[k] = (int)0x80000000; sb0.rmax[k] = 0; }
  sb0.n_refits = 0; sb0.pad = 0; sb0.pad2 = 0;
  MGF_TRY(h2d(ctx, G.sb.p, &sb0, 1));
  k_scene_bounds<<<std::min<unsigned>(nblk(nf), 256u), kBlock, 0, s>>>(G.fb_c.p, G.fb_r.p, (uint32_t)nf, G.sb.p);
  LAUNCH_CHECK();
  if (G.bits[0] + G.bits[1] + G.bits[2] == 0) return MGF_OK;
  k_morton_count<<<nblk(nf), kBlock, 0, s>>>(G.fb_c.p, (uint32_t)nf, G.sb.p, kMortonBits - 2 * (int)levels, G.cell_of.p, G.cell_rank.p, G.cell_cnt.p, 0.0f,
                                             make_uint3(G.bits[0], G.bits[1], G.bits[2]));
  LAUNCH_CHECK();
  MGF_TRY(prim_exclusive_scan_u32(ctx, G.cell_cnt.p, G.cell_lo.p, (size_t)cells + 1));
  FaceGrid FG = t->face_grid();
  k_scatter_leaves<<<nblk(nf), kBlock, 0, s>>>(FG.T, G.fb_c.p, G.fb_r.p, G.cell_of.p, G.cell_rank.p, G.brank.p, nullptr, nullptr, nullptr, nullptr, nullptr, 0.0f, 0.0f);
  LAUNCH_CHECK();
  MGF_HIP_TRY(hipStreamSynchronize(s));
  G.ready = true;
  return MGF_OK;
}

extern "C" mgf_status mgf_world_set_terrain(mgf_world* w, const mgf_mesh* mesh) {
  if (!w) return fail(MGF_ERR_INVALID, "world is NULL");
  w->invalidate_tick_caches();
  MGF_TRY(ctx_bind(w->ctx));
  if (!mesh) { w->terrain.reset(); return MGF_OK; }
  std::unique_ptr<mgf_mesh> t(new mgf_mesh());
  t->ctx = w->ctx;
  t->x = mesh->x;
  t->verts = mesh->verts;
  t->faces = mesh->faces;
  t->m.tree = mesh->m.tree;
  t->geom_version = 1;
  MGF_TRY(t->sync());
  MGF_TRY(build_face_grid(t.get()));
  w->terrain = std::move(t);
  w->terrain_grid_off = false;
  return MGF_OK;
}


extern "C" mgf_status mgf_world_add_obstacle(mgf_world* w, const mgf_compound* c) {
  if (!w || !c) return fail(MGF_ERR_INVALID, "NULL argument");
  if (w->obstacles.size() >= kObstacleMax) return fail(MGF_ERR_CAPACITY, "at most 256 obstacles");
  if (c->comps.size() >= kObstacleCompMax) return fail(MGF_ERR_CAPACITY, "an obstacle holds at most 2^18 components");
  MGF_TRY(ctx_bind(w->ctx));
  w->invalidate_tick_caches();
  std::unique_ptr<mgf_compound> o(new mgf_compound());
// ... 44 lines not shown
    Comp local = k; local.p = k.p + -px;
    M3 inv;
    if (!invert(tensor_of(local, mass[i]), &inv)) return fail(MGF_ERR_SINGULAR, "inertia tensor is not invertible (physics.rs:212)");
    float inv_mass = 1.0f / mass[i];
    V3 force = mk3(world_force[i].x, world_force[i].y, world_force[i].z) * mass[i];
    hx[i] = make_float4(px.x, px.y, px.z, 0.0f);
    hq[i] = make_float4(pq.s, pq.v.x, pq.v.y, pq.v.z);
    hs[4 * i] = make_float4(0, 0, 0, 0);
    hs[4 * i + 1] = make_float4(0, 0, inv_mass, inv.c[0].x);
    hs[4 * i + 2] = make_float4(inv.c[0].y, inv.c[0].z, inv.c[1].x, inv.c[1].y);
    hs[4 * i + 3] = make_float4(inv.c[1].z, inv.c[2].x, inv.c[2].y, inv.c[2].z);
    h0[i] = make_float4(force.x, force.y, force.z, restitution[i]);
    h1[i] = make_float4(0, 0, 0, friction[i]);
    uint32_t kind_bits = (uint32_t)k.kind;
    float kf; memcpy(&kf, &kind_bits, 4);
    hc[i] = make_float4(kf, k.r, half_h, 0.0f);
    for (int c = 0; c < 3; ++c) hi[3 * i + c] = make_float4(inv.c[c].x, inv.c[c].y, inv.c[c].z, 0.0f);
    hd[i] = make_float4(0, 0, 0, friction[i]);
    he[i] = make_float4(px.x, px.y, px.z, restitution[i]);
    c0[i] = make_float4(k.p.x, k.p.y, k.p.z, k.r);
    c1[i] = make_float4(k.d.x, k.d.y, k.d.z, kf);
    Box tb = swept_bounds(k, mk3(0, 0, 0));
    tc[i] = make_float4(tb.c.x, tb.c.y, tb.c.z, 0); tr[i] = make_float4(tb.r.x, tb.r.y, tb.r.z, 0);
    V3 fm = mk3(w->params.fat_margin, w->params.fat_margin, w->params.fat_margin);
    V3 frr = tb.r + fm;
    fc[i] = tc[i]; fr[i] = make_float4(frr.x, frr.y, frr.z, 0);
    w->shape_rmax[0] = std::max(w->shape_rmax[0], frr.x); w->shape_rmax[1] = std::max(w->shape_rmax[1], frr.y); w->shape_rmax[2] = std::max(w->shape_rmax[2], frr.z);
  }
  mgf_ctx* ctx = w->ctx;
  size_t o = w->n_owned;
  w->sbg_valid = false; w->ptrs_out = false;
  MGF_TRY(append(ctx, w->x, o, hx)); MGF_TRY(append(ctx, w->q, o, hq)); MGF_TRY(append(ctx, w->srec, 4 * o, hs));
  MGF_TRY(append(ctx, w->sp0, o, h0)); MGF_TRY(append(ctx, w->sp1, o, h1)); MGF_TRY(append(ctx, w->ctor, o, hc));
  MGF_TRY(append(ctx, w->imb, 3 * o, hi)); MGF_TRY(append(ctx, w->delta, o, hd)); MGF_TRY(append(ctx, w->einfo, o, he));
  MGF_TRY(append(ctx, w->col0, o, c0)); MGF_TRY(append(ctx, w->col1, o, c1)); MGF_TRY(append(ctx, w->tb_c, o, tc));
  MGF_TRY(append(ctx, w->tb_r, o, tr)); MGF_TRY(append(ctx, w->fb_c, o, fc)); MGF_TRY(append(ctx, w->fb_r, o, fr));
  if (w->has_compound) {
    std::vector<uint32_t> pz(N, 0u);
    std::vector<float4> fz(kMaxParts * N, make_float4(0, 0, 0, 0));
    MGF_TRY(append(ctx, w->pcount, o, pz));
    MGF_TRY(append(ctx, w->lp0, kMaxParts * o, fz)); MGF_TRY(append(ctx, w->lp1, kMaxParts * o, fz));
    MGF_TRY(append(ctx, w->wp0, kMaxParts * o, fz)); MGF_TRY(append(ctx, w->wp1, kMaxParts * o, fz));
  }
  w->n_owned += (uint32_t)n;
  w->n = w->n_owned;
  w->has_sphere = hs_; w->has_capsule = hc_;
  w->constraints_ready = false;
  return MGF_OK;
}

extern "C" mgf_status mgf_world_add_compound_bodies(mgf_world* w, const mgf_component* comps, const float* comp_mass, const int64_t* offsets,
                                                    int64_t n, const float* restitution, const float* friction, const mgf_vec3* world_force,
                                                    uint64_t* first_id) {
  if (!w || (n && (!comps || !comp_mass || !offsets || !restitution || !friction || !world_force))) return fail(MGF_ERR_INVALID, "NULL argument");
  MGF_TRY(world_identity(w));
  w->sidx_valid = false;
  w->invalidate_tick_caches();
  MGF_TRY(ctx_bind(w->ctx));
  w->n = w->n_owned;
  if (first_id) *first_id = w->n_owned;
  if (n <= 0) return MGF_OK;
  if ((uint64_t)w->n_owned + (uint64_t)n > 0x7FFFFFF0ull) return fail(MGF_ERR_INVALID, "too many bodies");
  const size_t N = (size_t)n, o = w->n_owned;
  std::vector<float4> hx(N), hq(N), hs(4 * N), h0(N), h1(N), hc(N), hi(3 * N), hd(N), he(N), c0(N), c1(N), tc(N), tr(N), fc(N), fr(N);
  std::vector<uint32_t> hp(N);
  std::vector<float4> l0(kMaxParts * N, make_float4(0, 0, 0, 0)), l1(l0), w0(l0), w1(l0);
  std::vector<float4> xa0, xa1, xb0, xb1;
  bool hs_ = w->has_sphere, hc_ = w->has_capsule;
// ... 41 lines not shown
    for (int64_t k = k0; k < k1; ++k) {
      const Comp& c = part[k - k0];
      uint32_t kb = (uint32_t)c.kind; float kbf; memcpy(&kbf, &kb, 4);
      const V3 lp = c.p + -com;
      if (k1 - k0 > kMaxParts) {
        if (k == k0) { const uint32_t off = w->x_used + (uint32_t)xa0.size(); float of; memcpy(&of, &off, 4); l0[kMaxParts * b] = make_float4(of, 0.0f, 0.0f, 0.0f); }
        xa0.push_back(make_float4(lp.x, lp.y, lp.z, c.r)); xa1.push_back(make_float4(c.d.x, c.d.y, c.d.z, kbf));
        xb0.push_back(make_float4(c.p.x, c.p.y, c.p.z, c.r)); xb1.push_back(make_float4(c.d.x, c.d.y, c.d.z, kbf));
      } else {
      l0[kMaxParts * b + (k - k0)] = make_float4(lp.x, lp.y, lp.z, c.r);
      l1[kMaxParts * b + (k - k0)] = make_float4(c.d.x, c.d.y, c.d.z, kbf);
      w0[kMaxParts * b + (k - k0)] = make_float4(c.p.x, c.p.y, c.p.z, c.r);
      w1[kMaxParts * b + (k - k0)] = make_float4(c.d.x, c.d.y, c.d.z, kbf);
      }
      Box pb = swept_bounds(c, mk3(0, 0, 0));
      tb = k == k0 ? pb : box_combine(tb, pb);
    }
    hp[b] = (uint32_t)(k1 - k0);
    tc[b] = make_float4(tb.c.x, tb.c.y, tb.c.z, 0); tr[b] = make_float4(tb.r.x, tb.r.y, tb.r.z, 0);
    const V3 fm = mk3(w->params.fat_margin, w->params.fat_margin, w->params.fat_margin), frr = tb.r + fm;
    fc[b] = tc[b]; fr[b] = make_float4(frr.x, frr.y, frr.z, 0);
    w->shape_rmax[0] = std::max(w->shape_rmax[0], frr.x); w->shape_rmax[1] = std::max(w->shape_rmax[1], frr.y); w->shape_rmax[2] = std::max(w->shape_rmax[2], frr.z);
  }
  mgf_ctx* ctx = w->ctx;
  if (!w->has_compound && o > 0) {
    std::vector<uint32_t> pz(o, 0u);
    std::vector<float4> fz(kMaxParts * o, make_float4(0, 0, 0, 0));
    MGF_TRY(append(ctx, w->pcount, 0, pz));
    MGF_TRY(append(ctx, w->lp0, 0, fz)); MGF_TRY(append(ctx, w->lp1, 0, fz)); MGF_TRY(append(ctx, w->wp0, 0, fz)); MGF_TRY(append(ctx, w->wp1, 0, fz));
  }
  w->sbg_valid = false; w->ptrs_out = false;
  MGF_TRY(append(ctx, w->x, o, hx)); MGF_TRY(append(ctx, w->q, o, hq)); MGF_TRY(append(ctx, w->srec, 4 * o, hs));
  MGF_TRY(append(ctx, w->sp0, o, h0)); MGF_TRY(append(ctx, w->sp1, o, h1)); MGF_TRY(append(ctx, w->ctor, o, hc));
  MGF_TRY(append(ctx, w->imb, 3 * o, hi)); MGF_TRY(append(ctx, w->delta, o, hd)); MGF_TRY(append(ctx, w->einfo, o, he));
  MGF_TRY(append(ctx, w->col0, o, c0)); MGF_TRY(append(ctx, w->col1, o, c1)); MGF_TRY(append(ctx, w->tb_c, o, tc));
  MGF_TRY(append(ctx, w->tb_r, o, tr)); MGF_TRY(append(ctx, w->fb_c, o, fc)); MGF_TRY(append(ctx, w->fb_r, o, fr));
  MGF_TRY(append(ctx, w->pcount, o, hp));
  MGF_TRY(append(ctx, w->lp0, kMaxParts * o, l0)); MGF_TRY(append(ctx, w->lp1, kMaxParts * o, l1));
  MGF_TRY(append(ctx, w->wp0, kMaxParts * o, w0)); MGF_TRY(append(ctx, w->wp1, kMaxParts * o, w1));
  if (!xa0.empty()) {
    MGF_TRY(append(ctx, w->xl0, w->x_used, xa0)); MGF_TRY(append(ctx, w->xl1, w->x_used, xa1));
    MGF_TRY(append(ctx, w->xw0, w->x_used, xb0)); MGF_TRY(append(ctx, w->xw1, w->x_used, xb1));
    w->x_used += (uint32_t)xa0.size();
  }
  w->has_compound = true;
  for (size_t b = 0; b < N; ++b) w->max_parts = std::max(w->max_parts, (uint32_t)(offsets[b + 1] - offsets[b]));
  w->n_owned += (uint32_t)n;
  w->n = w->n_owned;
  w->has_sphere = hs_; w->has_capsule = hc_;
  w->constraints_ready = false;
  return MGF_OK;
}

static mgf_status state_pin_ensure(mgf_world* w, size_t bytes) {
  if (w->state_pin_bytes >= bytes) return MGF_OK;
  if (w->state_pin) { (void)hipStreamSynchronize(w->ctx->stream); (void)hipHostFree(w->state_pin); w->state_pin = nullptr; w->state_pin_bytes = 0; }
  const size_t want = bytes + bytes / 4;
  MGF_HIP_TRY(hipHostMalloc(&w->state_pin, want, hipHostMallocDefault));
  w->state_pin_bytes = want;
  return MGF_OK;
}
extern "C" mgf_status mgf_world_read_state(mgf_world* w, mgf_vec3* x, mgf_quat* q, mgf_vec3* v, mgf_vec3* omega, mgf_vec3* delta, int64_t cap) {
  if (!w) return fail(MGF_ERR_INVALID, "world is NULL");
  MGF_TRY(ctx_bind(w->ctx));
  const size_t n = w->n_owned;
  if ((int64_t)n > cap) return fail(MGF_ERR_CAPACITY, "state buffers too small");
  if (n == 0) return MGF_OK;
  hipStream_t s = w->ctx->stream;
// ... 51 lines not shown
  MGF_HIP_TRY(hipStreamSynchronize(s));
  return MGF_OK;
}
extern "C" mgf_status mgf_world_read_colliders(mgf_world* w, mgf_moving_component* out, int64_t cap) {
  if (!w || !out) return fail(MGF_ERR_INVALID, "NULL argument");
  MGF_TRY(ctx_bind(w->ctx));
  size_t n = w->n_owned;
  if ((int64_t)n > cap) return fail(MGF_ERR_CAPACITY, "buffer too small");
  static_assert(sizeof(mgf_moving_component) == 44, "eleven 4-byte words, no padding: k_pack_colliders writes the struct as it lies");
  if (n == 0) return MGF_OK;
  hipStream_t s = w->ctx->stream;
  MGF_TRY(w->state_pack.ensure(11 * n, s));
  MGF_TRY(state_pin_ensure(w, 44 * n));
  k_pack_colliders<<<nblk(n), kBlock, 0, s>>>(w->bodies(), (uint32_t)n, w->permuted ? w->slot_of.p : nullptr, reinterpret_cast<uint32_t*>(w->state_pack.p));
  LAUNCH_CHECK();
  MGF_HIP_TRY(hipMemcpyAsync(w->state_pin, w->state_pack.p, 44 * n, hipMemcpyDeviceToHost, s));
  MGF_HIP_TRY(hipStreamSynchronize(s));
  memcpy(out, w->state_pin, 44 * n);
  return MGF_OK;
}
extern "C" mgf_status mgf_world_get(mgf_world* w, const mgf_body_ref* r, mgf_velocity* vel, mgf_rigid_body_info* info) {
  if (!w || !r) return fail(MGF_ERR_INVALID, "NULL argument");
  MGF_TRY(ctx_bind(w->ctx));
  if (r->tag == 1) {
    if (vel) { vel->linear = {0, 0, 0}; vel->angular = {0, 0, 0}; }
    if (info) { info->x = r->center; info->restitution = 0.0f; info->friction = r->friction; info->inv_mass = 0.0f; for (float& f : info->inv_moment) f = 0.0f; }
    return MGF_OK;
  }
  if (r->index >= w->n_owned) return fail(MGF_ERR_INVALID, "index out of bounds");
  MGF_TRY(perm_host(w));
  const size_t slot = w->permuted ? w->h_slot_of[r->index] : (size_t)r->index;
  float4 s[4], e, d;
  MGF_TRY(d2h(w->ctx, s, w->srec.p + 4 * slot, 4));
  MGF_TRY(d2h(w->ctx, &e, w->einfo.p + slot, 1));
  MGF_TRY(d2h(w->ctx, &d, w->delta.p + slot, 1));
  if (vel) { vel->linear = {s[0].x, s[0].y, s[0].z}; vel->angular = {s[0].w, s[1].x, s[1].y}; }
  if (info) {
    info->x = {e.x, e.y, e.z}; info->restitution = e.w; info->friction = d.w; info->inv_mass = s[1].z;
    float im[9] = {s[1].w, s[2].x, s[2].y, s[2].z, s[2].w, s[3].x, s[3].y, s[3].z, s[3].w};
    memcpy(info->inv_moment, im, sizeof(im));
  }
  return MGF_OK;
}
extern "C" mgf_status mgf_world_set(mgf_world* w, const mgf_body_ref* r, const mgf_velocity* vel) {
  if (!w || !r || !vel) return fail(MGF_ERR_INVALID, "NULL argument");
  MGF_TRY(ctx_bind(w->ctx));
  if (r->tag == 1) return MGF_OK;
  if (r->index >= w->n_owned) return fail(MGF_ERR_INVALID, "index out of bounds");
  MGF_TRY(perm_host(w));
  const size_t slot = w->permuted ? w->h_slot_of[r->index] : (size_t)r->index;
  float4 s[2];
  MGF_TRY(d2h(w->ctx, s, w->srec.p + 4 * slot, 2));
  s[0] = make_float4(vel->linear.x, vel->linear.y, vel->linear.z, vel->angular.x);
  s[1].x = vel->angular.y; s[1].y = vel->angular.z;
  return h2d(w->ctx, w->srec.p + 4 * slot, s, 2);
}
extern "C" mgf_status mgf_world_device_ptr(mgf_world* w, const char* name, void** ptr, int64_t* bytes) {
  if (!w || !name || !ptr) return fail(MGF_ERR_INVALID, "NULL argument");
  const size_t per = !strcmp(name, "x") || !strcmp(name, "q") || !strcmp(name, "delta") ? 16 : (!strcmp(name, "solver_rec") ? 64 : 0);
  if (!per) return fail(MGF_ERR_INVALID, "unknown array name");
  MGF_TRY(world_identity(w));
  w->invalidate_tick_caches();
  w->ptrs_out = true;
  *ptr = !strcmp(name, "x") ? (void*)w->x.p : !strcmp(name, "q") ? (void*)w->q.p : !strcmp(name, "delta") ? (void*)w->delta.p : (void*)w->srec.p;
  if (bytes) *bytes = (int64_t)(per * w->n_owned);
  return MGF_OK;
}
// ... 12 lines not shown
```

mgf_amd/csrc/k_bodies.h:

```cpp
#pragma once
#include <stddef.h>

#include <type_traits>

#include "dev_geom.h"
#include "host_bvh.h"

namespace mgf {

constexpr uint32_t kNone = 0xFFFFFFFFu;
constexpr int kBlock = 256;

__device__ __forceinline__ float4 ld4(const float4* p) { return *p; }
__device__ __forceinline__ V3 xyz(float4 v) { return mk3(v.x, v.y, v.z); }
__device__ __forceinline__ float4 mk4(V3 v, float w) { return make_float4(v.x, v.y, v.z, w); }
__device__ __forceinline__ float u2f(uint32_t u) { return __builtin_bit_cast(float, u); }
__device__ __forceinline__ uint32_t f2u(float f) { return __builtin_bit_cast(uint32_t, f); }

struct Bodies {
  float4* x;
  float4* q;
  float4* srec;
  float4* sp0;
  float4* sp1;
  float4* ctor;
  float4* imb;
  float4* delta;
  float4* einfo;
  float4* col0;
  float4* col1;
  float4* bpk;
  float4* tb_c;
  float4* tb_r;
  float4* fb_c;
  float4* fb_r;
  uint32_t* pcount;
  float4* lp0;
  float4* lp1;
  float4* wp0;
  float4* wp1;
  float4* xl0;
  float4* xl1;
  float4* xw0;
  float4* xw1;
};
constexpr int kMaxParts = 4;
constexpr int kBigParts = 32;
constexpr int kTileParts = 4;

constexpr int kBoundSlots = 64, kBoundSlotInts = 32;
struct SceneBounds { int lo[3]; int hi[3]; uint32_t n_refits; uint32_t pad; int rmax[3]; uint32_t pad2; };

__device__ __forceinline__ int f_ord(float f) { int i = __builtin_bit_cast(int, f); return i >= 0 ? i : (i ^ 0x7FFFFFFF); }
__host__ __device__ __forceinline__ float ord_f(int i) { int j = i >= 0 ? i : (i ^ 0x7FFFFFFF); return __builtin_bit_cast(float, j); }

__device__ __forceinline__ size_t part_at(const Bodies& B, uint32_t i, uint32_t k, uint32_t pc) {
  return pc > (uint32_t)kMaxParts ? (size_t)__builtin_bit_cast(uint32_t, B.lp0[(size_t)kMaxParts * i].x) + k : (size_t)kMaxParts * i + k;
}
__device__ __forceinline__ void world_part(const Bodies& B, uint32_t i, uint32_t k, uint32_t pc, float4& a, float4& b) {
  const size_t at = part_at(B, i, k, pc);
  if (pc > (uint32_t)kMaxParts) { a = B.xw0[at]; b = B.xw1[at]; } else { a = B.wp0[at]; b = B.wp1[at]; }
}
__device__ __forceinline__ M3 load_imb(const float4* imb, uint32_t i) {
  float4 a = imb[3 * i], b = imb[3 * i + 1], c = imb[3 * i + 2];
// ... 65 lines not shown
      v = v + xyz(p0) * inv_mass * dt;
      w = w + I * xyz(p1) * dt;
      int kind = (int)f2u(ct.x);
      V3 d = v * dt;
      Comp col;
      Box tb;
      const uint32_t pc = B.pcount ? B.pcount[i] : 0u;
      if (pc) {
        col.kind = KIND_SPHERE; col.p = x; col.d = mk3(0.0f, 0.0f, 0.0f); col.r = 0.0f;
        const bool big = pc > (uint32_t)kMaxParts;
        const size_t at0 = part_at(B, i, 0u, pc);
        const float4 *L0 = big ? B.xl0 : B.lp0, *L1 = big ? B.xl1 : B.lp1;
        float4 *W0 = big ? B.xw0 : B.wp0, *W1 = big ? B.xw1 : B.wp1;
        for (uint32_t k = 0; k < pc; ++k) {
          float4 l0 = L0[at0 + k], l1 = L1[at0 + k];
          Comp part; part.kind = (int)f2u(l1.w); part.r = l0.w;
          part.p = x + rotate(q, xyz(l0));
          part.d = part.kind == KIND_SPHERE ? mk3(0.0f, 0.0f, 0.0f) : rotate(q, xyz(l1));
          W0[at0 + k] = mk4(part.p, part.r);
          W1[at0 + k] = mk4(part.d, l1.w);
          Box pb = swept_bounds(part, d);
          tb = k == 0 ? pb : box_combine(tb, pb);
        }
      } else {
        col = construct(kind, ct.y, ct.z, x, q);
        tb = swept_bounds(col, d);
      }
      B.q[i] = make_float4(q.s, q.v.x, q.v.y, q.v.z);
      s_rec[wv][0 * 65 + lane] = make_float4(v.x, v.y, v.z, w.x);
      s_rec[wv][1 * 65 + lane] = make_float4(w.y, w.z, inv_mass, I.c[0].x);
      s_rec[wv][2 * 65 + lane] = make_float4(I.c[0].y, I.c[0].z, I.c[1].x, I.c[1].y);
      s_rec[wv][3 * 65 + lane] = make_float4(I.c[1].z, I.c[2].x, I.c[2].y, I.c[2].z);
      B.delta[i] = mk4(d, p1.w);
      B.einfo[i] = mk4(x + d, p0.w);
      B.col0[i] = mk4(col.p, col.r);
      B.col1[i] = mk4(col.d, u2f((uint32_t)col.kind));
      s_rec[wv][4 * 65 + lane] = mk4(col.p, col.r); s_rec[wv][5 * 65 + lane] = mk4(d, p1.w);
      s_rec[wv][6 * 65 + lane] = mk4(x + d, p0.w); s_rec[wv][7 * 65 + lane] = mk4(col.d, u2f((uint32_t)col.kind));
      B.tb_c[i] = mk4(tb.c, 0.0f);
      B.tb_r[i] = mk4(tb.r, 0.0f);
      Box fb; fb.c = xyz(B.fb_c[i]); fb.r = xyz(B.fb_r[i]);
      if (!box_contains(fb, tb)) {
        fb.c = tb.c;
        fb.r = tb.r + mk3(fat_margin, fat_margin, fat_margin);
        B.fb_c[i] = mk4(fb.c, 0.0f);
        B.fb_r[i] = mk4(fb.r, 0.0f);
        refit = true;
      }
      blo[0] = bhi[0] = f_ord(fb.c.x); blo[1] = bhi[1] = f_ord(fb.c.y); blo[2] = bhi[2] = f_ord(fb.c.z);
      brm[0] = f_ord(fb.r.x); brm[1] = f_ord(fb.r.y); brm[2] = f_ord(fb.r.z);
      if (wd.list && is_wide(wd.limit, mk4(fb.r, 0.0f))) {
        const uint32_t at = atomicAdd(wd.count, 1u);
        if (at < kWideCap) { wd.list[2 * at] = mk4(fb.c, u2f(i)); wd.list[2 * at + 1] = mk4(fb.r, u2f(wd.ext ? wd.ext[i] : i)); }
        blo[0] = blo[1] = blo[2] = 0x7FFFFFFF; bhi[0] = bhi[1] = bhi[2] = (int)0x80000000; brm[0] = brm[1] = brm[2] = 0;
      }
      if (cs.grid) {
        const uint32_t cell = morton_cell_of(fb.c, cs.grid, cs.min_frac, cs.shift);
        cs.cell_of[i] = cell;
        cs.rank[i] = atomicAdd(&cs.cell_cnt[cell], 1u);
      }
      tail(i, tb, s_tail, near_nt, near_pk);
      if (Tail::kNear && near_nt) { near0 = mk4(col.p, col.r); near1 = mk4(d, u2f(i)); }
    } else if (do_complete) {
      B.einfo[i] = mk4(x + xyz(dl), B.einfo[i].w);
    }
    if (do_complete) B.x[i] = mk4(x, 0.0f);
  }
  if (do_integrate) {
    __builtin_amdgcn_fence(__ATOMIC_ACQ_REL, "wavefront");
    const uint32_t i0 = blockIdx.x * kBlock + (uint32_t)wv * 64u;
#pragma unroll
    for (int it = 0; it < 4; ++it) {
      const int f = it * 64 + lane, rec = f >> 2, k = f & 3;
      if (i0 + (uint32_t)rec < n) {
        B.srec[4 * (size_t)i0 + f] = s_rec[wv][k * 65 + rec];
        if (B.bpk) B.bpk[4 * (size_t)i0 + f] = s_rec[wv][(4 + k) * 65 + rec];
      }
    }
  }
  if (!do_integrate || sb == nullptr) return;
  uint32_t near_rank = 0;
  if (Tail::kNear && near_nt) near_rank = atomicAdd(&s_near[0], 1u);
  int nref = __syncthreads_count(refit ? 1 : 0);
  if (threadIdx.x == 0 && nref) atomicAdd(&sb->n_refits, (uint32_t)nref);
  if (Tail::kNear && tail.near_list) {
    if (threadIdx.x == 0 && s_near[0]) s_near[1] = atomicAdd(tail.near_cnt, s_near[0]);
    __syncthreads();
    if (near_nt) {
      const size_t at = (size_t)s_near[1] + near_rank;
      tail.near_list[3 * at] = near0;
      tail.near_list[3 * at + 1] = near1;
      tail.near_list[3 * at + 2] = make_float4(u2f(near_nt), u2f((uint32_t)near_pk), u2f((uint32_t)(near_pk >> 32)), 0.0f);
    }
  }
  if (!sb_part) return;
  bounds_block_accumulate(blo, bhi, brm, sb_part);
}

__global__ __launch_bounds__(kBlock) void k_scene_bounds(const float4* fb_c, const float4* fb_r, uint32_t n, SceneBounds* sb) {
  int lo[3] = {0x7FFFFFFF, 0x7FFFFFFF, 0x7FFFFFFF}, hi[3] = {(int)0x80000000, (int)0x80000000, (int)0x80000000};
  int rm[3] = {0, 0, 0};
  for (uint32_t i = blockIdx.x * kBlock + threadIdx.x; i < n; i += gridDim.x * kBlock) {
    float4 c = fb_c[i], r = fb_r[i];
    int o[3] = {f_ord(c.x), f_ord(c.y), f_ord(c.z)};
    int e[3] = {f_ord(r.x), f_ord(r.y), f_ord(r.z)};
    for (int k = 0; k < 3; ++k) { lo[k] = min(lo[k], o[k]); hi[k] = max(hi[k], o[k]); rm[k] = max(rm[k], e[k]); }
  }
  __shared__ int s_lo[3][kBlock / 64], s_hi[3][kBlock / 64], s_rm[3][kBlock / 64];
  for (int k = 0; k < 3; ++k) {
    int a = lo[k], b = hi[k], c = rm[k];
    for (int off = 32; off > 0; off >>= 1) { a = min(a, __shfl_xor(a, off)); b = max(b, __shfl_xor(b, off)); c = max(c, __shfl_xor(c, off)); }
    if ((threadIdx.x & 63) == 0) { s_lo[k][threadIdx.x >> 6] = a; s_hi[k][threadIdx.x >> 6] = b; s_rm[k][threadIdx.x >> 6] = c; }
  }
  __syncthreads();
  if (threadIdx.x < 3) {
    int k = threadIdx.x, a = s_lo[k][0], b = s_hi[k][0], c = s_rm[k][0];
    for (int w = 1; w < kBlock / 64; ++w) { a = min(a, s_lo[k][w]); b = max(b, s_hi[k][w]); c = max(c, s_rm[k][w]); }
    atomicMin(&sb->lo[k], a);
    atomicMax(&sb->hi[k], b);
    atomicMax(&sb->rmax[k], c);
  }
}

__global__ __launch_bounds__(kBlock) void k_refresh_einfo(Bodies B, uint32_t n) {
  uint32_t i = blockIdx.x * kBlock + threadIdx.x;
  if (i < n) B.einfo[i] = mk4(xyz(B.x[i]) + xyz(B.delta[i]), B.einfo[i].w);
}
__device__ __forceinline__ void reset_step(SceneBounds* sb, uint32_t* err, uint32_t* guard, const uint32_t* prev_fail, int spec, int* sb_part, uint32_t* near_cnt) {
  if (near_cnt && threadIdx.x == 0) *near_cnt = 0u;
  if (spec && (*prev_fail || err[2])) { if (threadIdx.x == 0) *guard = 1u; return; }
  if (sb_part && threadIdx.x < kBoundSlots) {
    int* slot = sb_part + (size_t)threadIdx.x * kBoundSlotInts;
    for (int k = 0; k < 3; ++k) { slot[k] = 0x7FFFFFFF; slot[3 + k] = (int)0x80000000; slot[6 + k] = 0; }
  }
  if (threadIdx.x == 0) {
    *guard = 0u;
    for (int k = 0; k < 3; ++k) { sb->lo[k] = 0x7FFFFFFF; sb->hi[k] = (int)0x80000000; }
    sb->n_refits = 0; sb->pad = 0; sb->pad2 = 0;
    for (int k = 0; k < 3; ++k) sb->rmax[k] = 0;
    err[0] = 0; err[1] = 0; err[8] = 0;
  }
}
__global__ void k_reset_step(SceneBounds* sb, uint32_t* err, uint32_t* guard, const uint32_t* prev_fail, int spec, int* sb_part, uint32_t* near_cnt = nullptr) {
  reset_step(sb, err, guard, prev_fail, spec, sb_part, near_cnt);
}
struct ResetOne { SceneBounds* sb; uint32_t* err; uint32_t* guard; const uint32_t* prev_fail; int* sb_part; uint32_t* near_cnt; };
constexpr int kWorldBatch = 8;
struct ResetBatch { ResetOne t[kWorldBatch]; };
__global__ void k_reset_step_batch(ResetBatch A) {
  const ResetOne& R = A.t[blockIdx.x];
  reset_step(R.sb, R.err, R.guard, R.prev_fail, 0, R.sb_part, R.near_cnt);
}

}
```

mgf_amd/csrc/k_broadphase.h:

```cpp
#pragma once
#include "k_bodies.h"

namespace mgf {

__device__ __forceinline__ uint32_t expand10(uint32_t v) {
  v = (v * 0x00010001u) & 0xFF0000FFu;
  v = (v * 0x00000101u) & 0x0F00F00Fu;
  v = (v * 0x00000011u) & 0xC30C30C3u;
  v = (v * 0x00000005u) & 0x49249249u;
  return v;
}
__device__ __forceinline__ uint32_t morton_quant(float v, float lo, float hi) {
  float ext = hi - lo;
  float t = ext > 0.0f ? (v - lo) / ext : 0.0f;
  int qv = (int)(t * 1023.0f);
  return (uint32_t)(qv < 0 ? 0 : (qv > 1023 ? 1023 : qv));
}
__device__ __forceinline__ uint32_t face_cell(uint32_t cx, uint32_t cy, uint32_t cz, uint3 bits) {
  return (((cx << bits.y) | cy) << bits.z) | cz;
}
constexpr int kMortonBits = 30;
constexpr float kBodyGridMinFrac = 0.5f;
__device__ __forceinline__ void grid_box(const SceneBounds* sb, float min_frac, uint32_t P, float* lo, float* hi) {
  float ext = 0.0f;
// ... 329 lines not shown
  float4* ltb;
  uint32_t* cell_lo;
  const uint32_t* ext;
  uint32_t n;
  uint32_t levels;
  uint32_t* err;
  unsigned long long* dbg;
};
constexpr int kLdsQNodes = 341;
__host__ __device__ __forceinline__ uint32_t qlevel_offset(uint32_t l) { return ((1u << (2 * l)) - 1u) / 3u; }

__device__ __forceinline__ void box_min_max(V3& lo, V3& hi, V3 l, V3 h) {
  lo = mk3(fminf(lo.x, l.x), fminf(lo.y, l.y), fminf(lo.z, l.z));
  hi = mk3(fmaxf(hi.x, h.x), fmaxf(hi.y, h.y), fmaxf(hi.z, h.z));
}

__device__ __forceinline__ float pair_query_pad(const V3& c, const V3& r, float pad_abs) {
  return pad_abs + 1e-5f * (fabs_rs(c.x) + fabs_rs(c.y) + fabs_rs(c.z) + r.x + r.y + r.z);
}
__device__ __forceinline__ void pair_query_region(const V3& qc, const V3& qr, float pad, const SceneBounds* sb, const uint32_t* nb, uint32_t* ca, uint32_t* d,
                                                  float min_frac, const SceneBounds* box = nullptr) {
  float glo[3], ghi[3];
  grid_box(box ? box : sb, min_frac, nb[0] + nb[1] + nb[2], glo, ghi);
#pragma unroll
  for (int k = 0; k < 3; ++k) {
    float lo = glo[k], hi = ghi[k], rm = ord_f(sb->rmax[k]);
    float a = at(qc, k) - at(qr, k) - rm - pad, b = at(qc, k) + at(qr, k) + rm + pad;
    uint32_t c0 = morton_quant(a, lo, hi) >> (10u - nb[k]), c1 = morton_quant(b, lo, hi) >> (10u - nb[k]);
    ca[k] = c0; d[k] = c1 - c0 + 1u;
  }
}

__device__ __forceinline__ void scatter_leaf(uint32_t body, const Lbvh& T, const float4* fb_c, const float4* fb_r, const uint32_t* cell_of,
                                             const uint32_t* rank, uint32_t* brank, const float4* col0, const float4* delta, const float4* tb_c,
                                             const float4* tb_r, const SceneBounds* sb, float pad_abs, float min_frac, const SceneBounds* box = nullptr,
                                             float3 wide_limit = make_float3(0.0f, 0.0f, 0.0f), uint32_t n_owned = 0u) {
  if (body >= T.n) return;
  uint32_t p = T.cell_lo[cell_of[body]] + rank[body];
  LeafRec lr; lr.c = mk4(xyz(fb_c[body]), u2f(body)); lr.r = mk4(xyz(fb_r[body]), u2f(order_id(T.ext, body)));
  if (wide_limit.x > 0.0f && body < n_owned) { const float lim[3] = {wide_limit.x, wide_limit.y, wide_limit.z}; if (is_wide(lim, fb_r[body])) lr.r.w = u2f(0xFFFFFFFFu); }
  T.leaves[p] = lr;
  if (T.lcol) { T.lcol[2 * p] = col0[body]; T.lcol[2 * p + 1] = delta[body]; }
  if (T.ltb) {
    const float4 c = tb_c[body], r = tb_r[body];
    const uint32_t P = 2u * T.levels;
    const uint32_t nb[3] = {(P + 2u) / 3u, (P + 1u) / 3u, P / 3u};
    uint32_t ca[3], d[3];
    pair_query_region(xyz(c), xyz(r), pair_query_pad(xyz(c), xyz(r), pad_abs), sb, nb, ca, d, min_frac, box);
    T.ltb[2 * p] = mk4(xyz(c), u2f(ca[0] | (ca[1] << 10) | (ca[2] << 20)));
    T.ltb[2 * p + 1] = mk4(xyz(r), u2f(min(d[0], 1023u) | (min(d[1], 1023u) << 10) | (min(d[2], 1023u) << 20)));
  }
  T.sidx[p] = body;
  brank[body] = p;
}
__global__ __launch_bounds__(kBlock) void k_scatter_leaves(Lbvh T, const float4* fb_c, const float4* fb_r, const uint32_t* cell_of,
                                                           const uint32_t* rank, uint32_t* brank, const float4* col0, const float4* delta, const float4* tb_c,
                                                           const float4* tb_r, const SceneBounds* sb, float pad_abs, float min_frac, const SceneBounds* box = nullptr,
                                                           float3 wide_limit = make_float3(0.0f, 0.0f, 0.0f), uint32_t n_owned = 0u) {
  scatter_leaf(blockIdx.x * kBlock + threadIdx.x, T, fb_c, fb_r, cell_of, rank, brank, col0, delta, tb_c, tb_r, sb, pad_abs, min_frac, box, wide_limit, n_owned);
}

__global__ __launch_bounds__(kBlock) void k_lbvh_low(Lbvh T, float4* sub_lo, float4* sub_hi) {
  __shared__ float s_lo[3][kBlock], s_hi[3][kBlock];
  __shared__ uint32_t s_rng[2][kBlock];
  const int t = threadIdx.x;
  uint32_t g = blockIdx.x * kBlock + t;
  V3 lo = mk3(kInf, kInf, kInf), hi = mk3(-kInf, -kInf, -kInf);
  uint32_t b0 = T.cell_lo[g], b1 = T.cell_lo[g + 1];
  for (uint32_t p = b0; p < b1; ++p) {
    LeafRec lr = T.leaves[p];
    box_min_max(lo, hi, xyz(lr.c) - xyz(lr.r), xyz(lr.c) + xyz(lr.r));
  }
  s_lo[0][t] = lo.x; s_lo[1][t] = lo.y; s_lo[2][t] = lo.z;
  s_hi[0][t] = hi.x; s_hi[1][t] = hi.y; s_hi[2][t] = hi.z;
  s_rng[0][t] = b0; s_rng[1][t] = b1;
  __syncthreads();
  uint32_t lvl = T.levels;
  uint32_t first = blockIdx.x * kBlock;
  for (int w = kBlock / 4; w >= 1; w >>= 2) {
    lvl -= 1;
    first >>= 2;
    QNode nd;
    V3 ulo = mk3(kInf, kInf, kInf), uhi = mk3(-kInf, -kInf, -kInf);
    if (t < w) {
#pragma unroll
      for (int c = 0; c < 4; ++c) {
        V3 l = mk3(s_lo[0][4 * t + c], s_lo[1][4 * t + c], s_lo[2][4 * t + c]);
        V3 h = mk3(s_hi[0][4 * t + c], s_hi[1][4 * t + c], s_hi[2][4 * t + c]);
        bool leaf_level = (w == kBlock / 4);
// ... 310 lines not shown
            uint32_t gm = (uint32_t)(hb >> gbase) & 255u;
            if (hit) {
              uint32_t slot = np + __popc(gm & ((1u << sub) - 1u));
              if (slot < (uint32_t)kRowCap) row[slot] = j;
            }
            np += __popc(gm);
          }
          fresh = false;
          continue;
        }
        k = 4 * k + 1 + (uint32_t)c;
        ++lvl;
        fresh = true;
        continue;
      }
      if (lvl == 0) break;
      k = (k - 1) >> 2;
      --lvl;
      fresh = false;
    }
  }
  if (sub == 0) {
    p_cnt[i] = np;
    if (np > (uint32_t)kRowCap) atomicOr(overflow, 1u);
  }
}

__device__ __forceinline__ Comp load_comp(const Bodies& B, uint32_t i) {
  float4 c0 = B.col0[i], c1 = B.col1[i];
  Comp k; k.p = xyz(c0); k.r = c0.w; k.d = xyz(c1); k.kind = (int)f2u(c1.w);
  return k;
}
__device__ __forceinline__ Comp load_comp_moving(const Bodies& B, uint32_t i, V3* v) {
  float4 c0, c1, dl;
  if (B.bpk) { c0 = B.bpk[4 * (size_t)i]; dl = B.bpk[4 * (size_t)i + 1]; c1 = B.bpk[4 * (size_t)i + 3]; }
  else { c0 = B.col0[i]; c1 = B.col1[i]; dl = B.delta[i]; }
  Comp k; k.p = xyz(c0); k.r = c0.w; k.d = xyz(c1); k.kind = (int)f2u(c1.w);
  *v = xyz(dl);
  return k;
}

constexpr uint32_t kGridMaxCells = 512;
constexpr uint32_t kPairStatWords = 1024;

struct PairSrcGlobal {
  Lbvh T;
  __device__ __forceinline__ void range(uint32_t cell, const uint32_t*, uint32_t& p0, uint32_t& p1) const { p0 = T.cell_lo[cell]; p1 = T.cell_lo[cell + 1]; }
  __device__ __forceinline__ void leaf(uint32_t p, float4& c, float4& r) const { LeafRec lr = T.leaves[p]; c = lr.c; r = lr.r; }
  __device__ __forceinline__ void col(uint32_t p, float4& c0, float4& d0, uint32_t& j) const { c0 = T.lcol[2 * p]; d0 = T.lcol[2 * p + 1]; j = T.sidx[p]; }
};
template <bool SPHERES, class Src, class AccT>
__device__ __forceinline__ void pair_query_cells(const Src& S, const Box& q, const Comp& A, V3 vA, uint32_t oi , uint32_t n_owned, const uint32_t* ca,
                                                 const uint32_t* d, const uint32_t* nb, int shift, int sub, int gbase, uint32_t* row, AccT* acc,
                                                 uint32_t* overflow, uint32_t& np, uint32_t& n_accepted) {
  const uint32_t ncell = d[0] * d[1] * d[2];
  const uint32_t m2 = ((1u << 20) + d[2] - 1u) / d[2], m1 = ((1u << 20) + d[1] - 1u) / d[1];
  np = 0;
  for (uint32_t cb = 0; cb < ncell; cb += kCoopLanes) {
    uint32_t idx = cb + (uint32_t)sub;
    uint32_t p0 = 0, p1 = 0;
    if (idx < ncell) {
      const uint32_t t = (idx * m2) >> 20, cz = idx - t * d[2];
      const uint32_t cx = (t * m1) >> 20, cy = t - cx * d[1];
      const uint32_t cc3[3] = {ca[0] + cx, ca[1] + cy, ca[2] + cz};
      uint32_t code = (expand10(cc3[0] << (10u - nb[0])) << 2) | (expand10(cc3[1] << (10u - nb[1])) << 1) | expand10(cc3[2] << (10u - nb[2]));
      S.range(code >> shift, cc3, p0, p1);
    }
    for (;;) {
      bool more = p0 < p1;
// ... 509 lines not shown
```

mgf_amd/csrc/k_contacts.h:

```cpp
#pragma once
#include "k_broadphase.h"

namespace mgf {

struct NContact { float4 la, lb, n; };
struct RevEnt { uint32_t c, a, oid, pad; };
static_assert(sizeof(RevEnt) == 16, "a row entry is one 16-byte word");


template <int KA, int KB>
__global__ __launch_bounds__(kBlock) void k_narrow_pairs(Bodies B, const uint32_t* work, const uint32_t* m_ptr, const uint32_t* p_owner,
                                                         const uint32_t* p_cand, uint32_t* p_nc, NContact* p_out) {
  __shared__ uint32_t s_list[kBlock];
  __shared__ uint32_t s_n;
  if (threadIdx.x == 0) s_n = 0;
  __syncthreads();
  {
    const uint32_t t = blockIdx.x * kBlock + threadIdx.x;
    bool live = false;
    uint32_t p0 = 0;
    if (t < *m_ptr) {
      p0 = work ? work[t] : t;
      V3 v0, v1;
      Comp A0 = load_comp_moving(B, p_owner[p0], &v0), B0 = load_comp_moving(B, p_cand[p0], &v1);
// ... 600 lines not shown
                                                float dt, float baumgarte, float slop) {
  V3 t0, t1;
  compute_basis(normal, &t0, &t1);
  return make_constraint_basis(ia, ib, A, xa, rest_a, fric_a, Bd, xb, rest_b, fric_b, normal, t0, t1, ra, rb, dt, baumgarte, slop);
}

__device__ __forceinline__ void store_crec(CRec* dst, const CRec& c) {
  const float4* s = reinterpret_cast<const float4*>(&c);
  float4* d = reinterpret_cast<float4*>(dst);
#pragma unroll
  for (int k = 0; k < 8; ++k) d[k] = s[k];
}
__device__ __forceinline__ CRec load_crec(const CRec* src) {
  CRec c;
  const float4* s = reinterpret_cast<const float4*>(src);
  float4* d = reinterpret_cast<float4*>(&c);
#pragma unroll
  for (int k = 0; k < 8; ++k) d[k] = s[k];
  return c;
}
static_assert(offsetof(CRec, nimp) == 88 && offsetof(CRec, round) == 92 && offsetof(CRec, indeg) == 100, "CRec layout");
__device__ __forceinline__ CRec load_crec_solve(const CRec* src) {
  CRec c;
  const float4* s = reinterpret_cast<const float4*>(src);
  float4* d = reinterpret_cast<float4*>(&c);
#pragma unroll
  for (int k = 0; k < 6; ++k) d[k] = s[k];
  d[6] = make_float4(0, 0, 0, 0); d[7] = make_float4(0, 0, 0, 0);
  return c;
}

struct BodyPack { float4 c0, dl, ei; };
__device__ __forceinline__ BodyPack load_pack(const Bodies& B, uint32_t i, bool with_collider) {
  BodyPack P;
  if (B.bpk) { P.c0 = B.bpk[4 * i]; P.dl = B.bpk[4 * i + 1]; P.ei = B.bpk[4 * i + 2]; }
  else { P.c0 = with_collider ? B.col0[i] : make_float4(0, 0, 0, 0); P.dl = B.delta[i]; P.ei = B.einfo[i]; }
  return P;
}

struct TerrainSetup {
  TerrainDev M;
  const uint32_t *t_owner, *t_nc, *t_pre;
  const NContact* t_in;
  uint32_t in_stride;
  uint32_t blocks;
  const uint32_t* t_cand;
  const float4* obs_center;
};
__device__ __forceinline__ void setup_terrain_one(const Bodies& B, const TerrainSetup& T, const StepCounts* sc, uint32_t p, const uint32_t* base, float dt,
                                                  float baumgarte, float slop, CRec* cons, uint2* ab) {
  if (p >= sc->Mt) return;
  uint32_t nc = T.t_nc[p];
  if (nc == 0) return;
  uint32_t i = T.t_owner[p];
  BodyDyn A = load_dyn(B.srec, i), S = static_dyn();
  const BodyPack Pa = load_pack(B, i, false);
  float4 ea = Pa.ei;
  V3 center = mk3(T.M.x[0], T.M.x[1], T.M.x[2]);
  if (T.obs_center) { const uint32_t f = T.t_cand[p]; if (f & 0x80000000u) center = xyz(T.obs_center[(f >> 23) & 0xFFu]); }
  for (uint32_t k = 0; k < nc; ++k) {
    NContact in = T.t_in[(size_t)T.in_stride * p + k];
    CRec r = make_constraint(i, kNone, A, xyz(ea), ea.w, Pa.dl.w, S, center, 0.0f, 0.0f, xyz(in.n), xyz(in.la), xyz(in.lb), dt,
                             baumgarte, slop);
    store_crec(&cons[base[i] + T.t_pre[p] + k], r);
    ab[base[i] + T.t_pre[p] + k] = make_uint2(i, kNone);
  }
}

template <bool SPHERES>
// ... 55 lines not shown
  float4 ea = Pa.ei, eb = Pb.ei;
  for (uint32_t q = 0; q < nc; ++q) {
    const uint32_t c = base[i] + p_pre[p] + q;
    NContact k = p_in[(size_t)in_stride * p + q];
    CRec r = make_constraint(i, j, A, xyz(ea), ea.w, Pa.dl.w, Bd, xyz(eb), eb.w, Pb.dl.w, xyz(k.n), xyz(k.la), xyz(k.lb),
                             dt, baumgarte, slop);
    store_crec(&cons[c], r);
    ab[c] = make_uint2(i, j);
    uint32_t pos = atomicAdd(&degb[j], 1u);
    if (pos < rev_cap) rev[(size_t)j * rev_cap + pos] = RevEnt{c, i, order_id(ext, i), 0u};
    else *rev_flag = 1u;
  }
}

#ifndef MGF_CS_ENT_CAP
#define MGF_CS_ENT_CAP 1536
#endif
constexpr uint32_t kCsEntCap = MGF_CS_ENT_CAP;
constexpr uint32_t kCsSumStride = 32;
#ifndef MGF_TC_LANES
#define MGF_TC_LANES 4
#endif
constexpr int kTcLanes = MGF_TC_LANES;
constexpr uint32_t kTcMesh = 64;
struct TerrainContacts {
  TerrainDev M;
  const float4* near_list; const uint32_t* near_cnt;
  uint32_t n_faces, n_verts, cap_row_t, cap_t;
  const uint32_t* rows_t;
  uint32_t* sums;
  NContact* t_out;
  uint32_t *tcn, *tpos;
  const uint32_t* guard;
  const float4* col1;
  const uint32_t* pcount; const float4 *wp0, *wp1;
  uint32_t check; uint32_t* flag;
};
template <int GEN>
__device__ __forceinline__ void terrain_contacts_job(const TerrainContacts& A, uint32_t job_block, uint32_t job_blocks) {
  const TerrainDev& M = A.M;
  const float4* near_list = A.near_list; const uint32_t n_faces = A.n_faces, n_verts = A.n_verts, cap_row_t = A.cap_row_t, cap_t = A.cap_t;
  const uint32_t* rows_t = A.rows_t; uint32_t* sums = A.sums; NContact* t_out = A.t_out; uint32_t* tcn = A.tcn; uint32_t* tpos = A.tpos;
  __shared__ uint4 s_face[kTcMesh];
  __shared__ float4 s_vert[kTcMesh];
  const uint32_t L = *A.guard ? 0u : *A.near_cnt;
  const uint32_t per_pass = job_blocks * (uint32_t)(kBlock / kTcLanes);
  if (job_block * (uint32_t)(kBlock / kTcLanes) >= L) return;
  const bool staged = n_faces <= kTcMesh && n_verts <= kTcMesh;
  if (staged) {
    for (uint32_t e = threadIdx.x; e < n_faces; e += kBlock) s_face[e] = M.faces[e];
    for (uint32_t e = threadIdx.x; e < n_verts; e += kBlock) s_vert[e] = M.verts[e];
    __syncthreads();
  }
  const int lane = threadIdx.x & 63;
  const uint32_t sub = threadIdx.x % (uint32_t)kTcLanes;
  const V3 mx = mk3(M.x[0], M.x[1], M.x[2]);
  for (uint32_t e0 = job_block * (uint32_t)(kBlock / kTcLanes) + ((uint32_t)threadIdx.x & ~63u) / (uint32_t)kTcLanes; e0 < L; e0 += per_pass) {
    const uint32_t e = e0 + (uint32_t)lane / (uint32_t)kTcLanes;
    uint32_t i = 0, nt = 0, pk0 = 0, pk1 = 0;
    float4 r0 = make_float4(0, 0, 0, 0), r1 = r0;
    if (e < L) {
      r0 = near_list[3 * (size_t)e]; r1 = near_list[3 * (size_t)e + 1];
      const float4 r2 = near_list[3 * (size_t)e + 2];
      i = f2u(r1.w); nt = f2u(r2.x); pk0 = f2u(r2.y); pk1 = f2u(r2.z);
    }
    if (nt > cap_row_t) nt = 0;
    uint32_t run = 0, tp = 0;
// ... 92 lines not shown
        const uint32_t f = bytes ? ((a < 4u ? pk0 >> (8u * a) : pk1 >> (8u * (a - 4u))) & 255u) : rt[a];
        const uint4 fi = staged ? s_face[f] : M.faces[f];
        Triangle tri = staged ? mkt(xyz(s_vert[fi.x]) + mx, xyz(s_vert[fi.y]) + mx, xyz(s_vert[fi.z]) + mx)
                              : mkt(xyz(M.verts[fi.x]) + mx, xyz(M.verts[fi.y]) + mx, xyz(M.verts[fi.z]) + mx);
        Contact raw = mkc(mk3(0, 0, 0), mk3(0, 0, 0), mk3(0, 0, 0), 0.0f);
        const uint32_t nc = tri_msphere_x4(tri, mks(Ca.p, Ca.r), vA, &raw, (int)sub, lane & ~(kTcLanes - 1)) ? 1u : 0u;
        if (sub == 0u && tp + a < cap_t) {
          NContact o;
          o.la = make_float4(0, 0, 0, 0); o.lb = make_float4(0, 0, 0, u2f(0u)); o.n = make_float4(0, 0, 0, 0);
          if (nc) {
            const V3 a_c = comp_center(Ca) + vA * raw.t;
            const Contact g = neg(raw);
            o.la = mk4(raw.b + -a_c, g.t); o.lb = mk4(raw.a + -mx, u2f(1u)); o.n = mk4(g.n, 0.0f);
          }
          t_out[2 * (size_t)(tp + a)] = o;
        }
        run += nc;
      }
    }
    if (e < L && sub == 0u) {
      tcn[i] = run;
      tpos[i] = tp;
    }
    uint32_t wrun = sub == 0u ? run : 0u;
#pragma unroll
    for (int o = 32; o >= 1; o >>= 1) wrun += __shfl_xor(wrun, o);
    if (lane == 0 && wrun) atomicAdd(&sums[kCsSumStride], wrun);
  }
}
template <int GEN>
__global__ __launch_bounds__(kBlock) void k_terrain_contacts(TerrainContacts A) { terrain_contacts_job<GEN>(A, blockIdx.x, gridDim.x); }
template <int GEN>
__global__ __launch_bounds__(kBlock) void k_scatter_leaves_tc(Lbvh T, const float4* fb_c, const float4* fb_r, const uint32_t* cell_of,
                                                              const uint32_t* rank, uint32_t* brank, const float4* col0, const float4* delta, const float4* tb_c,
                                                              const float4* tb_r, const SceneBounds* sb, float pad_abs, float min_frac, TerrainContacts A, uint32_t tc_blocks,
                                                              const SceneBounds* box, float3 wide_limit, uint32_t n_owned) {
  if (blockIdx.x < tc_blocks) { terrain_contacts_job<GEN>(A, blockIdx.x, tc_blocks); return; }
  scatter_leaf((blockIdx.x - tc_blocks) * kBlock + threadIdx.x, T, fb_c, fb_r, cell_of, rank, brank, col0, delta, tb_c, tb_r, sb, pad_abs, min_frac, box, wide_limit, n_owned);
}
struct ContactsSpheres {
  const StepCounts* sc;
  uint32_t n, cap_row_t, cap_c, cap_t;
  const uint32_t *rows_p, *t_cnt, *p_cnt, *base, *tcn, *tpos;
  const NContact* t_out;
  float dt, baumgarte, slop;
  CRec* cons; uint2* ab; uint32_t* degb; RevEnt* rev; uint32_t rev_cap; uint32_t* rev_flag; uint32_t* flag;
  const uint32_t* ext;
  uint32_t t_blocks, region_cap, regions, cnt_stride;
  const uint32_t *slot_body, *slot_cnt;
};
__device__ __forceinline__ void cs_list_row(const uint32_t* rp, uint32_t np, const uint32_t* ext, uint32_t first, uint32_t w0, uint32_t owner, uint32_t* s_j, uint16_t* s_b) {
  if (np <= 12u) {
    uint32_t pj[12], o_id[12];
#pragma unroll
    for (int a = 0; a < 12; a += 4) {
      uint4 v = make_uint4(0, 0, 0, 0);
      if ((uint32_t)a < np) v = *reinterpret_cast<const uint4*>(rp + a);
      pj[a] = v.x; pj[a + 1] = v.y; pj[a + 2] = v.z; pj[a + 3] = v.w;
    }
#pragma unroll
    for (int a = 0; a < 12; ++a) o_id[a] = (uint32_t)a < np ? order_id(ext, pj[a]) : 0xFFFFFFFFu;
#pragma unroll
    for (int a = 0; a < 12; ++a) {
      uint32_t before = 0;
#pragma unroll
      for (int q = 0; q < 12; ++q) before += o_id[q] < o_id[a] ? 1u : 0u;
      const uint32_t pos = first + before - w0;
      if ((uint32_t)a < np && pos < kCsEntCap) { s_j[pos] = pj[a]; s_b[pos] = (uint16_t)owner; }
    }
  } else {
    for (uint32_t a = 0; a < np; ++a) {
      const uint32_t j = rp[a], oa = order_id(ext, j);
      uint32_t before = 0;
      for (uint32_t q = 0; q < np; ++q) before += order_id(ext, rp[q]) < oa ? 1u : 0u;
      const uint32_t pos = first + before - w0;
      if (pos < kCsEntCap) { s_j[pos] = j; s_b[pos] = (uint16_t)owner; }
    }
  }
}
__device__ __attribute__((noinline)) void cs_list_row_again(const uint32_t* rp, uint32_t np, const uint32_t* ext, uint32_t first, uint32_t w0, uint32_t owner,
                                                            uint32_t* s_j, uint16_t* s_b) {
  for (uint32_t a = 0; a < np; ++a) {
    const uint32_t j = rp[a], oa = order_id(ext, j);
    uint32_t before = 0;
    for (uint32_t q = 0; q < np; ++q) before += order_id(ext, rp[q]) < oa ? 1u : 0u;
    const uint32_t pos = first + before - w0;
    if (pos < kCsEntCap) { s_j[pos] = j; s_b[pos] = (uint16_t)owner; }
  }
}
template <bool SPH>
__device__ __forceinline__ Comp pack_comp(const Bodies& B, uint32_t i, const BodyPack& P) {
  Comp X; X.p = xyz(P.c0); X.r = P.c0.w; X.d = mk3(0.0f, 0.0f, 0.0f); X.kind = KIND_SPHERE;
  if (!SPH) { const float4 c1 = B.bpk ? B.bpk[4 * (size_t)i + 3] : B.col1[i]; X.d = xyz(c1); X.kind = (int)f2u(c1.w); }
  return X;
}
template <bool SPH>
__global__ __launch_bounds__(kBlock) void k_contacts_rows(Bodies B, TerrainDev M, ContactsSpheres A) {
  __shared__ float4 s_w[kBlock / 64][7 * 65];
  __shared__ uint32_t s_c[kBlock / 64][64];
  __shared__ uint32_t s_j[kCsEntCap];
  __shared__ uint16_t s_b[kCsEntCap];
  __shared__ uint32_t s_cbase[kBlock];
  __shared__ uint32_t s_wave[kBlock / 64];
  if (A.sc->fail) return;
  if (blockIdx.x < A.t_blocks) {
    const uint32_t p = blockIdx.x * (uint32_t)kBlock + threadIdx.x, region = p / A.region_cap;
    if (region >= A.regions || p - region * A.region_cap >= min(A.slot_cnt[region * A.cnt_stride], A.region_cap)) return;
    const NContact in0 = A.t_out[2 * (size_t)p];
    const uint32_t nc = f2u(in0.lb.w);
    if (nc == 0) return;
    const uint32_t i = A.slot_body[p], tp = A.tpos[i];
    uint32_t c = A.base[i];
    for (uint32_t q = tp; q < p; ++q) c += f2u(A.t_out[2 * (size_t)q].lb.w);
    const V3 mx = mk3(M.x[0], M.x[1], M.x[2]);
    const BodyDyn Ad = load_dyn(B.srec, i), S = static_dyn();
    const BodyPack Pa = load_pack(B, i, false);
    for (uint32_t k = 0; k < nc; ++k, ++c) {
      const NContact in = k == 0 ? in0 : A.t_out[2 * (size_t)p + k];
      const CRec r = make_constraint(i, kNone, Ad, xyz(Pa.ei), Pa.ei.w, Pa.dl.w, S, mx, 0.0f, 0.0f, xyz(in.n), xyz(in.la), xyz(in.lb), A.dt, A.baumgarte, A.slop);
      store_crec(&A.cons[c], r);
      A.ab[c] = make_uint2(i, kNone);
    }
    return;
  }
  const int t = threadIdx.x, lane = t & 63, wv = t >> 6;
  const uint32_t i0 = (blockIdx.x - A.t_blocks) * (uint32_t)kBlock, i = i0 + (uint32_t)t;
// ... 99 lines not shown
```

mgf_amd/csrc/k_tiles.h:

```cpp
#pragma once
#include "k_solver_flow6.h"

namespace mgf {

constexpr int kGhostFloats = 40 + 8 * kTileParts;
constexpr int kGhostFloatsPlain = 40;

constexpr int kTileBatch = 8;
struct SelTile {
  const float4 *fb_c, *fb_r, *x;
  uint32_t n;
  float x_left, x_right, x_lo, x_hi;
  uint32_t* blk;
  uint32_t* tot;
  uint32_t* tot_host;
  uint32_t *ids_l, *ids_r, *ids_m;
};
struct SelBatch { SelTile t[kTileBatch]; };
__device__ __forceinline__ uint32_t sel_flags(const SelTile& S, uint32_t i) {
  const float c = S.fb_c[i].x, h = S.fb_r[i].x, cx = S.x[i].x;
  uint32_t f = 0;
  if (c - h < S.x_left) f |= 1u;
  if (c + h > S.x_right) f |= 2u;
  if (cx < S.x_lo) f |= 4u; else if (cx >= S.x_hi) f |= 8u;
// ... 101 lines not shown
  for (uint32_t k = 0; k < 10; ++k) put(k, r[k]);
  if (rec <= (uint32_t)kGhostFloatsPlain) return;
  for (uint32_t k = 0; k < (uint32_t)kTileParts; ++k) {
    float4 a = make_float4(0, 0, 0, 0), b = a;
    if (k < pc) { a = B.wp0[kMaxParts * i + k]; b = B.wp1[kMaxParts * i + k]; }
    put(10 + 2 * k, a); put(11 + 2 * k, b);
  }
}
struct ExpTile { Bodies B; const uint32_t *ids_l, *ids_r; uint32_t nl, nr; float* out; uint32_t rec, pad; };
struct ExpBatch { ExpTile t[kTileBatch]; };
__global__ __launch_bounds__(kBlock) void k_export_bodies(ExpBatch A) {
  const ExpTile& E = A.t[blockIdx.y];
  const uint32_t t = blockIdx.x * kBlock + threadIdx.x;
  if (t >= E.nl + E.nr) return;
  export_body(E.B, t < E.nl ? E.ids_l[t] : E.ids_r[t - E.nl], E.out + (size_t)t * E.rec, E.rec);
}
__device__ __forceinline__ void import_ghost(Bodies B, uint32_t i, const float* src, float fat_margin, int blo[3], int bhi[3], int brm[3], uint32_t rec = (uint32_t)kGhostFloats) {
  const bool vec = (reinterpret_cast<uintptr_t>(src) & 15u) == 0u;
  auto get = [&](uint32_t k) -> float4 {
    if (vec) return reinterpret_cast<const float4*>(src)[k];
    return make_float4(src[4 * k], src[4 * k + 1], src[4 * k + 2], src[4 * k + 3]);
  };
  float o[40];
#pragma unroll
  for (uint32_t k = 0; k < 10; ++k) { const float4 v = get(k); o[4 * k] = v.x; o[4 * k + 1] = v.y; o[4 * k + 2] = v.z; o[4 * k + 3] = v.w; }
  V3 x = mk3(o[0], o[1], o[2]), d = mk3(o[13], o[14], o[15]);
  B.x[i] = mk4(x, 0.0f);
  B.q[i] = make_float4(o[3], o[4], o[5], o[6]);
  B.srec[4 * i] = make_float4(o[7], o[8], o[9], o[10]);
  B.srec[4 * i + 1] = make_float4(o[11], o[12], o[24], o[25]);
  B.srec[4 * i + 2] = make_float4(o[26], o[27], o[28], o[29]);
  B.srec[4 * i + 3] = make_float4(o[30], o[31], o[32], o[33]);
  B.delta[i] = mk4(d, o[35]);
  B.einfo[i] = mk4(x + d, o[34]);
  Comp k; k.kind = (int)f2u(o[16]); k.p = mk3(o[17], o[18], o[19]); k.d = mk3(o[20], o[21], o[22]); k.r = o[23];
  B.col0[i] = mk4(k.p, k.r);
  B.col1[i] = mk4(k.d, o[16]);
  if (B.bpk) { B.bpk[4 * i] = mk4(k.p, k.r); B.bpk[4 * i + 1] = mk4(d, o[35]); B.bpk[4 * i + 2] = mk4(x + d, o[34]); B.bpk[4 * i + 3] = mk4(k.d, o[16]); }
  Box tb = swept_bounds(k, d);
  const bool parts_in = rec > (uint32_t)kGhostFloatsPlain;
  const uint32_t pc = parts_in ? min(f2u(o[36]), (uint32_t)kTileParts) : 0u;
  if (B.pcount) {
    B.pcount[i] = pc;
    for (uint32_t pk = 0; pk < (uint32_t)kMaxParts; ++pk) {
      float4 a = make_float4(0, 0, 0, 0), b = a;
      if (parts_in && pk < (uint32_t)kTileParts) { a = get(10 + 2 * pk); b = get(11 + 2 * pk); }
      B.wp0[kMaxParts * i + pk] = a; B.wp1[kMaxParts * i + pk] = b;
      B.lp0[kMaxParts * i + pk] = a; B.lp1[kMaxParts * i + pk] = b;
      if (pk < pc) {
        Comp part; part.kind = (int)f2u(b.w); part.p = xyz(a); part.r = a.w; part.d = xyz(b);
        Box pb = swept_bounds(part, d);
        tb = pk == 0 ? pb : box_combine(tb, pb);
      }
    }
  }
  B.tb_c[i] = mk4(tb.c, 0.0f); B.tb_r[i] = mk4(tb.r, 0.0f);
  const V3 fr = tb.r + mk3(fat_margin, fat_margin, fat_margin);
  B.fb_c[i] = mk4(tb.c, 0.0f); B.fb_r[i] = mk4(fr, 0.0f);
  blo[0] = bhi[0] = f_ord(tb.c.x); blo[1] = bhi[1] = f_ord(tb.c.y); blo[2] = bhi[2] = f_ord(tb.c.z);
  brm[0] = f_ord(fr.x); brm[1] = f_ord(fr.y); brm[2] = f_ord(fr.z);
  B.sp0[i] = make_float4(0, 0, 0, o[34]); B.sp1[i] = make_float4(0, 0, 0, o[35]);
  B.ctor[i] = make_float4(pc ? u2f(2u) : o[16], k.r, 0.0f, 0.0f);
  B.imb[3 * i] = make_float4(0, 0, 0, 0); B.imb[3 * i + 1] = make_float4(0, 0, 0, 0); B.imb[3 * i + 2] = make_float4(0, 0, 0, 0);
}
struct ImpTile { Bodies B; uint32_t n_owned, m, m1; float fat_margin; const float *in, *in2; int* sb_part; uint32_t rec1, rec2; };
struct ImpBatch { ImpTile t[kTileBatch]; };
__global__ __launch_bounds__(kBlock) void k_import_ghosts(ImpBatch A) {
  const ImpTile& I = A.t[blockIdx.y];
  if (blockIdx.x * kBlock >= I.m) return;
  const uint32_t t = blockIdx.x * kBlock + threadIdx.x;
  int blo[3] = {0x7FFFFFFF, 0x7FFFFFFF, 0x7FFFFFFF}, bhi[3] = {(int)0x80000000, (int)0x80000000, (int)0x80000000}, brm[3] = {0, 0, 0};
// ... 42 lines not shown
__global__ __launch_bounds__(16 * kTileBatch) void k_fetch_flags(FlagBatch A) {
  const FlagTile& F = A.t[threadIdx.x >> 4];
  if ((threadIdx.x & 15u) < F.words) F.dst[threadIdx.x & 15u] = F.src[threadIdx.x & 15u];
}
constexpr int kTickSnapWords = 7;
struct SnapTile { Bodies B; uint32_t n, pad; float4* snap; };
struct SnapBatch { SnapTile t[kTileBatch]; };
__global__ __launch_bounds__(kBlock) void k_tick_snapshot(SnapBatch A, int restore) {
  const Bodies& B = A.t[blockIdx.y].B;
  const uint32_t n = A.t[blockIdx.y].n;
  float4* snap = A.t[blockIdx.y].snap;
  const uint32_t i = blockIdx.x * kBlock + threadIdx.x;
  if (i >= n) return;
  float4* s = snap + i;
  const size_t n_ = n;
  if (!restore) {
    s[0] = B.x[i]; s[n_] = B.q[i]; s[2 * n_] = B.srec[4 * (size_t)i]; s[3 * n_] = B.srec[4 * (size_t)i + 1]; s[4 * n_] = B.delta[i]; s[5 * n_] = B.fb_c[i]; s[6 * n_] = B.fb_r[i];
  } else {
    B.x[i] = s[0]; B.q[i] = s[n_]; B.srec[4 * (size_t)i] = s[2 * n_]; B.srec[4 * (size_t)i + 1] = s[3 * n_]; B.delta[i] = s[4 * n_]; B.fb_c[i] = s[5 * n_]; B.fb_r[i] = s[6 * n_];
  }
}
constexpr int kMigrantWords = 21 + 4 * kTileParts;
constexpr int kBodyWords = 21 + 4 * kMaxParts;
__device__ __forceinline__ float4* body_word(const Bodies& B, uint32_t e, uint32_t i) {
  switch (e) {
    case 0: return B.x + i;
    case 1: return B.q + i;
    case 2: case 3: case 4: case 5: return B.srec + 4 * (size_t)i + (e - 2);
    case 6: return B.sp0 + i;
    case 7: return B.sp1 + i;
    case 8: return B.ctor + i;
    case 9: case 10: case 11: return B.imb + 3 * (size_t)i + (e - 9);
    case 12: return B.delta + i;
    case 13: return B.einfo + i;
    case 14: return B.col0 + i;
    case 15: return B.col1 + i;
    case 16: return B.tb_c + i;
    case 17: return B.tb_r + i;
    case 18: return B.fb_c + i;
    default: return B.fb_r + i;
  }
}
__device__ __forceinline__ float4* part_word(const Bodies& B, uint32_t arr, uint32_t slot, uint32_t i) {
  float4* base = arr == 0 ? B.lp0 : (arr == 1 ? B.lp1 : (arr == 2 ? B.wp0 : B.wp1));
  return base + (size_t)kMaxParts * i + slot;
}
__device__ __forceinline__ float4 migrant_get(const Bodies& B, uint32_t e, uint32_t i, uint32_t slots) {
  if (e < 20u) return *body_word(B, e, i);
  if (!B.pcount) return make_float4(0, 0, 0, 0);
  if (e == 20u) return make_float4(u2f(B.pcount[i]), 0, 0, 0);
  const uint32_t k = e - 21u;
  return *part_word(B, k / slots, k % slots, i);
}
__device__ __forceinline__ void migrant_put(const Bodies& B, uint32_t e, uint32_t i, float4 v, uint32_t slots) {
  if (e < 20u) { *body_word(B, e, i) = v; return; }
  if (!B.pcount) return;
  if (e == 20u) { B.pcount[i] = f2u(v.x); return; }
  const uint32_t k = e - 21u, arr = k / slots, slot = k % slots;
  *part_word(B, arr, slot, i) = v;
  if (slots < (uint32_t)kMaxParts && slot + 1u == slots)
    for (uint32_t z = slots; z < (uint32_t)kMaxParts; ++z) *part_word(B, arr, z, i) = make_float4(0, 0, 0, 0);
}
__global__ __launch_bounds__(kBlock) void k_export_migrants(Bodies B, const uint32_t* ids, uint32_t m, float4* out, uint32_t slots) {
  const uint32_t words = 21u + 4u * slots;
  uint32_t t = blockIdx.x * kBlock + threadIdx.x;
  if (t >= m * words) return;
  uint32_t b = t / words, e = t % words;
  out[t] = migrant_get(B, e, ids[b], slots);
}
// ... 128 lines not shown
    const float ext = hi_f - lo_f;
    float t = ext > 0.0f ? (v - lo_f) / ext : 0.0f;
    t = t < 0.0f ? 0.0f : (t > 1.0f ? 1.0f : t);
    return (uint32_t)(t * (float)((1u << kPartCoordBits) - 1u));
  };
  const uint32_t cb = P.cb[axis];
  const uint32_t q = ((quant(axis) >> (kPartCoordBits - cb)) << (kPartCoordBits - cb)) | (quant((axis + 1) % 3) >> cb);
  keys[p] = (unit << kPartCoordBits) | q;
  if (vals_out) vals_out[p] = b;
}
__global__ __launch_bounds__(kBlock) void k_part_keys_block(uint32_t n, const uint32_t* vals, const float4* fb_c, const SceneBounds* sb, uint32_t nb,
                                                            uint32_t* keys) {
  const uint32_t p = blockIdx.x * kBlock + threadIdx.x;
  if (p >= n) return;
  const float4 c = fb_c[vals[p]];
  uint32_t code = 0;
#pragma unroll
  for (int k = 0; k < 3; ++k) code |= expand10(morton_quant(k == 0 ? c.x : (k == 1 ? c.y : c.z), ord_f(sb->lo[k]), ord_f(sb->hi[k])) >> 3) << (2 - k);
  keys[p] = ((p / nb) << 21) | (code & 0x1FFFFFu);
}

__global__ __launch_bounds__(kBlock) void k_iota(uint32_t* a, uint32_t n) {
  const uint32_t k = blockIdx.x * kBlock + threadIdx.x;
  if (k < n) a[k] = k;
}
__global__ __launch_bounds__(kBlock) void k_permute_ids(uint32_t n, const uint32_t* order, const uint32_t* old_ext, uint32_t* new_ext, uint32_t* slot_of) {
  const uint32_t k = blockIdx.x * kBlock + threadIdx.x;
  if (k >= n) return;
  const uint32_t o = order[k], e = old_ext ? old_ext[o] : o;
  new_ext[k] = e;
  slot_of[e] = k;
}

__global__ __launch_bounds__(kBlock) void k_kind_mask(const float4* col1, const uint32_t* pcount, uint32_t base, uint32_t m, uint32_t* mask) {
  uint32_t t = blockIdx.x * kBlock + threadIdx.x;
  if (t >= m) return;
  const uint32_t pc = pcount ? pcount[base + t] : 0u;
  atomicOr(mask, pc ? (pc > 2u ? 12u : 4u) : (f2u(col1[base + t].w) == (uint32_t)KIND_SPHERE ? 1u : 2u));
}
__global__ __launch_bounds__(kBlock) void k_record_max_parts(const float* rec, uint32_t m, uint32_t stride_floats, uint32_t at, uint32_t* out) {
  uint32_t t = blockIdx.x * kBlock + threadIdx.x;
  if (t < m) { const uint32_t pc = f2u(rec[(size_t)t * stride_floats + at]); if (pc) atomicMax(out, pc); }
}
__global__ __launch_bounds__(kBlock) void k_tags_set(float4* ctor, const uint32_t* tags, uint32_t n) {
  uint32_t i = blockIdx.x * kBlock + threadIdx.x;
  if (i < n) ctor[i].w = u2f(tags[i]);
}
__global__ __launch_bounds__(kBlock) void k_tags_get(const float4* ctor, uint32_t* tags, uint32_t n) {
  uint32_t i = blockIdx.x * kBlock + threadIdx.x;
  if (i < n) tags[i] = f2u(ctor[i].w);
}

}
```

mgf_amd/csrc/mgf_hip.hip:

```cpp
#include <stdarg.h>

#include <algorithm>
#include <cmath>
#include <memory>
#include <utility>

#include "common.h"
#include "kernels.h"
#include "scene_io.h"

using namespace mgf;

static thread_local char g_err[512] = "";
namespace mgf {
void set_error(const char* fmt, ...) {
  va_list ap;
  va_start(ap, fmt);
  vsnprintf(g_err, sizeof(g_err), fmt, ap);
  va_end(ap);
}
}
extern "C" const char* mgf_last_error(void) { return g_err; }
extern "C" const char* mgf_version(void) { return "mgf-hip 0.1 (gfx950)"; }
extern "C" mgf_params mgf_default_params(void) {
// ... 63 lines not shown
  if (ctx->stream) (void)hipStreamSynchronize(ctx->stream);
  ctx->closed = true;
  if (!ctx->own_stream) ctx->stream = nullptr;
  ctx_release(ctx);
}

static mgf_status ctx_bind(mgf_ctx* ctx) {
  if (!ctx) return fail(MGF_ERR_HIP, "no device context: this entry point computes on the GPU (mgf-hip has no CPU fallback)");
  if (ctx->closed) return fail(MGF_ERR_INVALID, "the context was destroyed (mgf_ctx_destroy): its handles can only be freed");
  MGF_HIP_TRY(hipSetDevice(ctx->device));
  (void)hipGetLastError();
  return MGF_OK;
}
template <class T>
static mgf_status h2d(mgf_ctx* ctx, T* dst, const T* src, size_t n) {
  if (n == 0) return MGF_OK;
  MGF_HIP_TRY(hipMemcpyAsync(dst, src, n * sizeof(T), hipMemcpyHostToDevice, ctx->stream));
  MGF_HIP_TRY(hipStreamSynchronize(ctx->stream));
  return MGF_OK;
}
template <class T>
static mgf_status d2h(mgf_ctx* ctx, T* dst, const T* src, size_t n) {
  if (n == 0) return MGF_OK;
  MGF_HIP_TRY(hipMemcpyAsync(dst, src, n * sizeof(T), hipMemcpyDeviceToHost, ctx->stream));
  MGF_HIP_TRY(hipStreamSynchronize(ctx->stream));
  return MGF_OK;
}

template <class T>
static mgf_status append(mgf_ctx* ctx, DBuf<T>& buf, size_t old_n, const std::vector<T>& add) {
  MGF_TRY(buf.ensure(old_n + add.size(), ctx->stream, true, old_n));
  return h2d(ctx, buf.p + old_n, add.data(), add.size());
}

extern "C" mgf_status mgf_exclusive_scan_u32(mgf_ctx* ctx, const uint32_t* in, int64_t n, uint32_t* out) {
  MGF_TRY(ctx_bind(ctx));
  if (n < 0 || (n && (!in || !out))) return fail(MGF_ERR_INVALID, "bad argument");
  if (n == 0) return MGF_OK;
  DBuf<uint32_t> d_in, d_out;
  MGF_TRY(d_in.ensure((size_t)n, ctx->stream)); MGF_TRY(d_out.ensure((size_t)n, ctx->stream));
  MGF_TRY(h2d(ctx, d_in.p, in, (size_t)n));
  MGF_TRY(prim_exclusive_scan_u32(ctx, d_in.p, d_out.p, (size_t)n));
  return d2h(ctx, out, d_out.p, (size_t)n);
}

#include "host_trees.inc"
#include "host_geom_io.inc"
#include "host_single_shot.inc"
#include "host_world.inc"
#include "host_perm.inc"
#include "host_tick.inc"
#include "host_tiles.inc"
#include "host_solver.inc"
#include "host_boundary.inc"
#include "host_tiles_native.inc"
#include "host_query.inc"
```

Measured before the change: 8.448 billion.

## Make packed body record the sole storage for collider and extent fields

Removes the separate einfo, col0 and col1 arrays and stores those fields only in the interleaved bpk record, accessed through PackField views. This drops the duplicate writes during integration and import, along with the runtime branch on whether the pack is valid. A small k_pack_motion kernel refreshes the delta slot when the pack does not cover all bodies. The cost is that every reader now goes through strided packed accesses, and a pack-off fallback no longer exists.

After: 8.500 billion, median of 6. About the same (+0.6%).

```diff
diff --git a/mgf_amd/csrc/host_boundary.inc b/mgf_amd/csrc/host_boundary.inc
--- a/mgf_amd/csrc/host_boundary.inc
+++ b/mgf_amd/csrc/host_boundary.inc
@@ -109,8 +109,8 @@
   const size_t n = src->n_owned;
   MGF_TRY(clone_buf(ctx, w->x, src->x, n)); MGF_TRY(clone_buf(ctx, w->q, src->q, n)); MGF_TRY(clone_buf(ctx, w->srec, src->srec, 4 * n));
   MGF_TRY(clone_buf(ctx, w->sp0, src->sp0, n)); MGF_TRY(clone_buf(ctx, w->sp1, src->sp1, n)); MGF_TRY(clone_buf(ctx, w->ctor, src->ctor, n));
-  MGF_TRY(clone_buf(ctx, w->imb, src->imb, 3 * n)); MGF_TRY(clone_buf(ctx, w->delta, src->delta, n)); MGF_TRY(clone_buf(ctx, w->einfo, src->einfo, n));
-  MGF_TRY(clone_buf(ctx, w->col0, src->col0, n)); MGF_TRY(clone_buf(ctx, w->col1, src->col1, n)); MGF_TRY(clone_buf(ctx, w->tb_c, src->tb_c, n));
+  MGF_TRY(clone_buf(ctx, w->imb, src->imb, 3 * n)); MGF_TRY(clone_buf(ctx, w->delta, src->delta, n)); MGF_TRY(clone_buf(ctx, w->bpk, src->bpk, 4 * n));
+  MGF_TRY(clone_buf(ctx, w->tb_c, src->tb_c, n));
   MGF_TRY(clone_buf(ctx, w->tb_r, src->tb_r, n)); MGF_TRY(clone_buf(ctx, w->fb_c, src->fb_c, n)); MGF_TRY(clone_buf(ctx, w->fb_r, src->fb_r, n));
   if (src->has_compound) {
     MGF_TRY(clone_buf(ctx, w->pcount, src->pcount, n));
@@ -138,7 +138,7 @@
   w->opt_solver_mode = src->opt_solver_mode; w->opt_two_pass = src->opt_two_pass; w->opt_broadphase_tree = src->opt_broadphase_tree;
   w->opt_terrain_tree = src->opt_terrain_tree; w->opt_no_fused_narrowphase = src->opt_no_fused_narrowphase;
   w->opt_no_fused_scene_bounds = src->opt_no_fused_scene_bounds; w->opt_no_fused_terrain_rows = src->opt_no_fused_terrain_rows;
-  w->opt_pair_brick = src->opt_pair_brick; w->opt_body_pack = src->opt_body_pack; w->opt_grid_min_frac_pct = src->opt_grid_min_frac_pct;
+  w->opt_pair_brick = src->opt_pair_brick; w->opt_grid_min_frac_pct = src->opt_grid_min_frac_pct;
   w->grid_occupancy = src->grid_occupancy;
   w->opt_cell_fill = src->opt_cell_fill; w->opt_cell_fill_set = src->opt_cell_fill_set; w->opt_pipeline = src->opt_pipeline; w->opt_spin_wait = src->opt_spin_wait; w->opt_readback_kernel = src->opt_readback_kernel;
   w->opt_stream_ordered = src->opt_stream_ordered; w->opt_flow_blocks_per_cu = src->opt_flow_blocks_per_cu; w->opt_flow_sleep = src->opt_flow_sleep;
diff --git a/mgf_amd/csrc/host_tick.inc b/mgf_amd/csrc/host_tick.inc
--- a/mgf_amd/csrc/host_tick.inc
+++ b/mgf_amd/csrc/host_tick.inc
@@ -11,7 +11,6 @@
   const uint32_t* guard = with_bounds ? w->scalars.p + 14 : nullptr;
   int* sb_part = (with_terrain_rows && integrate && with_bounds && !w->opt_no_fused_scene_bounds) ? w->sb_part.p : nullptr;
   w->bounds_cover = sb_part ? w->n_owned : 0u;
-  MGF_TRY(w->bpk.ensure(4 * (size_t)std::max(w->n, w->n_owned), ctx->stream));
   w->pack_cover = integrate ? w->n_owned : 0u;
   CellSort cs;
   memset(&cs, 0, sizeof(cs));
@@ -58,11 +57,10 @@
   return MGF_OK;
 }
 
-static mgf_status launch_pairs(mgf_world* w, int ka, int kb, const uint32_t* work, const uint32_t* m_ptr, uint32_t cap, bool pack_ok) {
+static mgf_status launch_pairs(mgf_world* w, int ka, int kb, const uint32_t* work, const uint32_t* m_ptr, uint32_t cap) {
   if (cap == 0) return MGF_OK;
   hipStream_t s = w->ctx->stream;
   Bodies B = w->bodies();
-  if (!pack_ok) B.bpk = nullptr;
   unsigned g = nblk(cap);
   if (ka == 0 && kb == 0) k_narrow_pairs<0, 0><<<g, kBlock, 0, s>>>(B, work, m_ptr, w->p_owner.p, w->p_cand.p, w->p_nc.p, w->p_out.p);
   else if (ka == 0 && kb == 1) k_narrow_pairs<0, 1><<<g, kBlock, 0, s>>>(B, work, m_ptr, w->p_owner.p, w->p_cand.p, w->p_nc.p, w->p_out.p);
@@ -71,11 +69,10 @@
   LAUNCH_CHECK();
   return MGF_OK;
 }
-static mgf_status launch_terrain(mgf_world* w, int ka, const TerrainDev& M, const uint32_t* work, const uint32_t* m_ptr, uint32_t cap, bool pack_ok) {
+static mgf_status launch_terrain(mgf_world* w, int ka, const TerrainDev& M, const uint32_t* work, const uint32_t* m_ptr, uint32_t cap) {
   if (cap == 0) return MGF_OK;
   hipStream_t s = w->ctx->stream;
   Bodies B = w->bodies();
-  if (!pack_ok) B.bpk = nullptr;
   unsigned g = nblk(cap);
   if (ka == 0) k_narrow_terrain<0><<<g, kBlock, 0, s>>>(B, M, work, m_ptr, w->t_owner.p, w->t_cand.p, w->t_nc.p, w->t_out.p);
   else k_narrow_terrain<1><<<g, kBlock, 0, s>>>(B, M, work, m_ptr, w->t_owner.p, w->t_cand.p, w->t_nc.p, w->t_out.p);
@@ -312,11 +309,13 @@
   w->plan.zero_launched = false;
   const bool bounds_done = w->bounds_cover == n && n > 0;
   const bool rows_done = w->terrain_rows_done;
-  const bool pack_ok = w->pack_cover == n && n > 0 && w->opt_body_pack;
+  if (w->pack_cover != n) {
+    k_pack_motion<<<nblk(n), kBlock, 0, s>>>(B, n);
+    LAUNCH_CHECK();
+  }
   if (!cleared) MGF_TRY(collide_prepare(w, solver_follows, false, false));
   const uint32_t cap_t = w->cap_t, cap_p = w->cap_p, cap_c = w->cap_c;
   const uint32_t levels = w->plan.levels, cells = w->plan.cells, nblocks = cells / kBlock;
-  if (!pack_ok) B.bpk = nullptr;
   const bool cells_done = cleared && bounds_done && w->cells_cover == n && w->cells_levels == w->plan.levels;
   w->invalidate_tick_caches();
   const bool fold_in_morton = cleared && bounds_done;
@@ -426,7 +425,7 @@
     A.n_faces = (uint32_t)(w->terrain->faces.size() / 3); A.n_verts = (uint32_t)w->terrain->verts.size(); A.cap_row_t = w->row_cap_t; A.cap_t = cap_t;
     A.rows_t = w->rows_t.p; A.sums = w->cs_sums.p; A.t_out = w->t_out.p; A.tcn = w->tcn.p; A.tpos = w->tpos.p; A.guard = w->scalars.p + 14;
     A.check = (front_rows && w->opt_front_rows_check) ? 1u : 0u; A.flag = w->d_err() + 8;
-    A.col1 = w->col1.p; A.pcount = w->has_compound ? w->pcount.p : nullptr; A.wp0 = w->wp0.p; A.wp1 = w->wp1.p;
+    A.col1 = B.col1; A.pcount = w->has_compound ? w->pcount.p : nullptr; A.wp0 = w->wp0.p; A.wp1 = w->wp1.p;
     const unsigned tg = std::max(1u, std::min(nblk((size_t)w->n_owned * kTcLanes / 8 + 1), 256u));
     if (front_rows) {
       hipStream_t ts = s;
@@ -445,16 +444,16 @@
       else k_terrain_contacts<1><<<tg, kBlock, 0, ts>>>(A);
       LAUNCH_CHECK();
       if (forked) MGF_HIP_TRY(hipEventRecord(w->ts->ev_join, ts));
-      k_scatter_leaves<<<nblk(n), kBlock, 0, s>>>(T, w->fb_c.p, w->fb_r.p, w->cell_of.p, w->cell_rank.p, w->brank.p, w->col0.p, w->delta.p, w->tb_c.p, w->tb_r.p, w->sb.p, 1e-3f, min_frac, grid_box_of, wlim, w->n_owned);
+      k_scatter_leaves<<<nblk(n), kBlock, 0, s>>>(T, w->fb_c.p, w->fb_r.p, w->cell_of.p, w->cell_rank.p, w->brank.p, w->bodies().col0, w->delta.p, w->tb_c.p, w->tb_r.p, w->sb.p, 1e-3f, min_frac, grid_box_of, wlim, w->n_owned);
     } else if (w->opt_fused_contacts >= 2) {
       k_terrain_contacts<0><<<tg, kBlock, 0, s>>>(A);
       LAUNCH_CHECK();
-      k_scatter_leaves<<<nblk(n), kBlock, 0, s>>>(T, w->fb_c.p, w->fb_r.p, w->cell_of.p, w->cell_rank.p, w->brank.p, w->col0.p, w->delta.p, w->tb_c.p, w->tb_r.p, w->sb.p, 1e-3f, min_frac, grid_box_of, wlim, w->n_owned);
+      k_scatter_leaves<<<nblk(n), kBlock, 0, s>>>(T, w->fb_c.p, w->fb_r.p, w->cell_of.p, w->cell_rank.p, w->brank.p, w->bodies().col0, w->delta.p, w->tb_c.p, w->tb_r.p, w->sb.p, 1e-3f, min_frac, grid_box_of, wlim, w->n_owned);
     } else {
-      k_scatter_leaves_tc<0><<<nblk(n) + tg, kBlock, 0, s>>>(T, w->fb_c.p, w->fb_r.p, w->cell_of.p, w->cell_rank.p, w->brank.p, w->col0.p, w->delta.p, w->tb_c.p, w->tb_r.p, w->sb.p, 1e-3f, min_frac, A, tg, grid_box_of, wlim, w->n_owned);
+      k_scatter_leaves_tc<0><<<nblk(n) + tg, kBlock, 0, s>>>(T, w->fb_c.p, w->fb_r.p, w->cell_of.p, w->cell_rank.p, w->brank.p, w->bodies().col0, w->delta.p, w->tb_c.p, w->tb_r.p, w->sb.p, 1e-3f, min_frac, A, tg, grid_box_of, wlim, w->n_owned);
     }
   } else {
-    k_scatter_leaves<<<nblk(n), kBlock, 0, s>>>(T, w->fb_c.p, w->fb_r.p, w->cell_of.p, w->cell_rank.p, w->brank.p, w->col0.p, w->delta.p, w->tb_c.p, w->tb_r.p, w->sb.p, 1e-3f, min_frac, grid_box_of, wlim, w->n_owned);
+    k_scatter_leaves<<<nblk(n), kBlock, 0, s>>>(T, w->fb_c.p, w->fb_r.p, w->cell_of.p, w->cell_rank.p, w->brank.p, w->bodies().col0, w->delta.p, w->tb_c.p, w->tb_r.p, w->sb.p, 1e-3f, min_frac, grid_box_of, wlim, w->n_owned);
   }
   LAUNCH_CHECK();
   w->sidx_valid = n == w->n_owned;
@@ -599,19 +598,19 @@
     }
   } else if (!mixed) {
     int k = w->has_capsule ? 1 : 0;
-    if (!fused) MGF_TRY(launch_pairs(w, k, k, nullptr, &sc->Mp, cap_p, pack_ok));
-    if (M.n_nodes || n_obs) MGF_TRY(launch_terrain(w, k, M, nullptr, &sc->Mt, cap_t, pack_ok));
+    if (!fused) MGF_TRY(launch_pairs(w, k, k, nullptr, &sc->Mp, cap_p));
+    if (M.n_nodes || n_obs) MGF_TRY(launch_terrain(w, k, M, nullptr, &sc->Mt, cap_t));
   } else {
     MGF_TRY(w->work_lists.ensure(4 * (size_t)cap_p + 2 * (size_t)cap_t, s));
     uint32_t* lists_p = w->work_lists.p;
     uint32_t* lists_t = w->work_lists.p + 4 * (size_t)cap_p;
     k_bin_pairs<<<nblk(cap_p), kBlock, 0, s>>>(B, &sc->Mp, cap_p, w->p_owner.p, w->p_cand.p, lists_p, sc->bins);
     LAUNCH_CHECK();
-    for (int ty = 0; ty < 4; ++ty) MGF_TRY(launch_pairs(w, ty >> 1, ty & 1, lists_p + (size_t)ty * cap_p, &sc->bins[ty], cap_p, pack_ok));
+    for (int ty = 0; ty < 4; ++ty) MGF_TRY(launch_pairs(w, ty >> 1, ty & 1, lists_p + (size_t)ty * cap_p, &sc->bins[ty], cap_p));
     if (M.n_nodes || n_obs) {
       k_bin_terrain<<<nblk(cap_t), kBlock, 0, s>>>(B, &sc->Mt, cap_t, w->t_owner.p, lists_t, sc->bins + 4);
       LAUNCH_CHECK();
-      for (int ty = 0; ty < 2; ++ty) MGF_TRY(launch_terrain(w, ty, M, lists_t + (size_t)ty * cap_t, &sc->bins[4 + ty], cap_t, pack_ok));
+      for (int ty = 0; ty < 2; ++ty) MGF_TRY(launch_terrain(w, ty, M, lists_t + (size_t)ty * cap_t, &sc->bins[4 + ty], cap_t));
     }
   }
   if (n_obs && cap_t) {
diff --git a/mgf_amd/csrc/host_tiles.inc b/mgf_amd/csrc/host_tiles.inc
--- a/mgf_amd/csrc/host_tiles.inc
+++ b/mgf_amd/csrc/host_tiles.inc
@@ -102,11 +102,10 @@
   if (need > 0x7FFFFFF0ull) return fail(MGF_ERR_INVALID, "too many bodies");
   MGF_TRY(grow_keep(w, w->x, 1, need)); MGF_TRY(grow_keep(w, w->q, 1, need)); MGF_TRY(grow_keep(w, w->srec, 4, need));
   MGF_TRY(grow_keep(w, w->sp0, 1, need)); MGF_TRY(grow_keep(w, w->sp1, 1, need)); MGF_TRY(grow_keep(w, w->ctor, 1, need));
-  MGF_TRY(grow_keep(w, w->imb, 3, need)); MGF_TRY(grow_keep(w, w->delta, 1, need)); MGF_TRY(grow_keep(w, w->einfo, 1, need));
-  MGF_TRY(grow_keep(w, w->col0, 1, need)); MGF_TRY(grow_keep(w, w->col1, 1, need)); MGF_TRY(grow_keep(w, w->tb_c, 1, need));
+  MGF_TRY(grow_keep(w, w->imb, 3, need)); MGF_TRY(grow_keep(w, w->delta, 1, need)); MGF_TRY(grow_keep(w, w->bpk, 4, need));
+  MGF_TRY(grow_keep(w, w->tb_c, 1, need));
   MGF_TRY(grow_keep(w, w->tb_r, 1, need)); MGF_TRY(grow_keep(w, w->fb_c, 1, need)); MGF_TRY(grow_keep(w, w->fb_r, 1, need));
   MGF_TRY(grow_parts(w, need));
-  MGF_TRY(grow_keep(w, w->bpk, 4, need));
   w->pack_cover = (w->pack_cover >= w->n_owned && w->n_owned > 0) ? (uint32_t)need : 0u;
   if (n_ghost > 0) {
     const bool join = w->bounds_cover == w->n_owned && w->n == w->n_owned && w->n_owned > 0;
@@ -232,8 +231,8 @@
   if (!kinds_hint) MGF_TRY(raise_parts_for_records(w, src, n_in, 4u * (uint32_t)kMigrantWords, 4u * 20u));
   MGF_TRY(grow_keep(w, w->x, 1, need)); MGF_TRY(grow_keep(w, w->q, 1, need)); MGF_TRY(grow_keep(w, w->srec, 4, need));
   MGF_TRY(grow_keep(w, w->sp0, 1, need)); MGF_TRY(grow_keep(w, w->sp1, 1, need)); MGF_TRY(grow_keep(w, w->ctor, 1, need));
-  MGF_TRY(grow_keep(w, w->imb, 3, need)); MGF_TRY(grow_keep(w, w->delta, 1, need)); MGF_TRY(grow_keep(w, w->einfo, 1, need));
-  MGF_TRY(grow_keep(w, w->col0, 1, need)); MGF_TRY(grow_keep(w, w->col1, 1, need)); MGF_TRY(grow_keep(w, w->tb_c, 1, need));
+  MGF_TRY(grow_keep(w, w->imb, 3, need)); MGF_TRY(grow_keep(w, w->delta, 1, need)); MGF_TRY(grow_keep(w, w->bpk, 4, need));
+  MGF_TRY(grow_keep(w, w->tb_c, 1, need));
   MGF_TRY(grow_keep(w, w->tb_r, 1, need)); MGF_TRY(grow_keep(w, w->fb_c, 1, need)); MGF_TRY(grow_keep(w, w->fb_r, 1, need));
   MGF_TRY(grow_parts(w, need));
   k_import_migrants<<<nblk((size_t)n_in * kMigrantWords), kBlock, 0, w->ctx->stream>>>(w->bodies(), w->n_owned, (uint32_t)n_in,
@@ -250,7 +249,7 @@
   }
   MGF_TRY(w->mig_cnt.ensure(2, w->ctx->stream));
   MGF_HIP_TRY(hipMemsetAsync(w->mig_cnt.p, 0, 8, w->ctx->stream));
-  k_kind_mask<<<nblk(n_in), kBlock, 0, w->ctx->stream>>>(w->col1.p, w->has_compound ? w->pcount.p : nullptr, w->n_owned - (uint32_t)n_in, (uint32_t)n_in, w->mig_cnt.p);
+  k_kind_mask<<<nblk(n_in), kBlock, 0, w->ctx->stream>>>(w->bodies().col1, w->has_compound ? w->pcount.p : nullptr, w->n_owned - (uint32_t)n_in, (uint32_t)n_in, w->mig_cnt.p);
   LAUNCH_CHECK();
   uint32_t mask = 0;
   MGF_TRY(d2h(w->ctx, &mask, w->mig_cnt.p, 1));
diff --git a/mgf_amd/csrc/host_world.inc b/mgf_amd/csrc/host_world.inc
--- a/mgf_amd/csrc/host_world.inc
+++ b/mgf_amd/csrc/host_world.inc
@@ -16,7 +16,7 @@
   DBuf<float4> mig_tmp;
   DBuf<float> state_pack;
   void* state_pin = nullptr; size_t state_pin_bytes = 0;
-  DBuf<float4> x, q, srec, sp0, sp1, ctor, imb, delta, einfo, col0, col1, tb_c, tb_r, fb_c, fb_r;
+  DBuf<float4> x, q, srec, sp0, sp1, ctor, imb, delta, tb_c, tb_r, fb_c, fb_r;
   DBuf<float4> bpk;
   DBuf<uint32_t> ext_of, ext_new, slot_of;
   DBuf<float4> perm_tmp;
@@ -71,7 +71,6 @@
   int64_t opt_front_rows_check = 0;
   bool front_rows_off = false;
   int64_t opt_fused_contacts = 1;
-  int64_t opt_body_pack = 1;
   int64_t opt_pair_brick = 1;
   uint64_t pair_brick_slow = 0;
   uint32_t pair_brick_off = 0;
@@ -240,7 +239,7 @@
   Bodies bodies() {
     Bodies B;
     B.x = x.p; B.q = q.p; B.srec = srec.p; B.sp0 = sp0.p; B.sp1 = sp1.p; B.ctor = ctor.p; B.imb = imb.p; B.bpk = bpk.p; B.delta = delta.p;
-    B.einfo = einfo.p; B.col0 = col0.p; B.col1 = col1.p; B.tb_c = tb_c.p; B.tb_r = tb_r.p; B.fb_c = fb_c.p; B.fb_r = fb_r.p;
+    B.einfo.pk = bpk.p; B.col0.pk = bpk.p; B.col1.pk = bpk.p; B.tb_c = tb_c.p; B.tb_r = tb_r.p; B.fb_c = fb_c.p; B.fb_r = fb_r.p;
     B.pcount = has_compound ? pcount.p : nullptr; B.lp0 = lp0.p; B.lp1 = lp1.p; B.wp0 = wp0.p; B.wp1 = wp1.p;
     B.xl0 = xl0.p; B.xl1 = xl1.p; B.xw0 = xw0.p; B.xw1 = xw1.p;
     return B;
@@ -382,7 +381,6 @@
     w->opt_flow_max_blocks = value; w->flow_grid = 0; w->flowk_grid = 0; w->flow5_prepped = false; w->flow6_prepped = false;
     return MGF_OK;
   }
-  if (!strcmp(key, "body_pack")) { w->opt_body_pack = value; return MGF_OK; }
   if (!strcmp(key, "grid_min_frac_pct")) { if (value < 0 || value > 100) return fail(MGF_ERR_INVALID, "grid_min_frac_pct: 0..100"); w->opt_grid_min_frac_pct = value; return MGF_OK; }
   if (!strcmp(key, "cell_fill")) { if (value < 1 || value > 1024) return fail(MGF_ERR_INVALID, "cell_fill out of range"); w->opt_cell_fill = value; w->opt_cell_fill_set = true; return MGF_OK; }
   if (!strcmp(key, "no_fused_scene_bounds")) { w->opt_no_fused_scene_bounds = value; return MGF_OK; }
@@ -648,7 +646,7 @@
   LAUNCH_CHECK();
   MGF_TRY(prim_exclusive_scan_u32(ctx, G.cell_cnt.p, G.cell_lo.p, (size_t)cells + 1));
   FaceGrid FG = t->face_grid();
-  k_scatter_leaves<<<nblk(nf), kBlock, 0, s>>>(FG.T, G.fb_c.p, G.fb_r.p, G.cell_of.p, G.cell_rank.p, G.brank.p, nullptr, nullptr, nullptr, nullptr, nullptr, 0.0f, 0.0f);
+  k_scatter_leaves<<<nblk(nf), kBlock, 0, s>>>(FG.T, G.fb_c.p, G.fb_r.p, G.cell_of.p, G.cell_rank.p, G.brank.p, PackField<0>{nullptr}, nullptr, nullptr, nullptr, nullptr, 0.0f, 0.0f);
   LAUNCH_CHECK();
   MGF_HIP_TRY(hipStreamSynchronize(s));
   G.ready = true;
@@ -759,8 +757,8 @@
   w->sbg_valid = false; w->ptrs_out = false;
   MGF_TRY(append(ctx, w->x, o, hx)); MGF_TRY(append(ctx, w->q, o, hq)); MGF_TRY(append(ctx, w->srec, 4 * o, hs));
   MGF_TRY(append(ctx, w->sp0, o, h0)); MGF_TRY(append(ctx, w->sp1, o, h1)); MGF_TRY(append(ctx, w->ctor, o, hc));
-  MGF_TRY(append(ctx, w->imb, 3 * o, hi)); MGF_TRY(append(ctx, w->delta, o, hd)); MGF_TRY(append(ctx, w->einfo, o, he));
-  MGF_TRY(append(ctx, w->col0, o, c0)); MGF_TRY(append(ctx, w->col1, o, c1)); MGF_TRY(append(ctx, w->tb_c, o, tc));
+  MGF_TRY(append(ctx, w->imb, 3 * o, hi)); MGF_TRY(append(ctx, w->delta, o, hd)); MGF_TRY(append(ctx, w->bpk, 4 * o, pack_records(c0, hd, he, c1)));
+  MGF_TRY(append(ctx, w->tb_c, o, tc));
   MGF_TRY(append(ctx, w->tb_r, o, tr)); MGF_TRY(append(ctx, w->fb_c, o, fc)); MGF_TRY(append(ctx, w->fb_r, o, fr));
   if (w->has_compound) {
     std::vector<uint32_t> pz(N, 0u);
@@ -868,8 +866,8 @@
   w->sbg_valid = false; w->ptrs_out = false;
   MGF_TRY(append(ctx, w->x, o, hx)); MGF_TRY(append(ctx, w->q, o, hq)); MGF_TRY(append(ctx, w->srec, 4 * o, hs));
   MGF_TRY(append(ctx, w->sp0, o, h0)); MGF_TRY(append(ctx, w->sp1, o, h1)); MGF_TRY(append(ctx, w->ctor, o, hc));
-  MGF_TRY(append(ctx, w->imb, 3 * o, hi)); MGF_TRY(append(ctx, w->delta, o, hd)); MGF_TRY(append(ctx, w->einfo, o, he));
-  MGF_TRY(append(ctx, w->col0, o, c0)); MGF_TRY(append(ctx, w->col1, o, c1)); MGF_TRY(append(ctx, w->tb_c, o, tc));
+  MGF_TRY(append(ctx, w->imb, 3 * o, hi)); MGF_TRY(append(ctx, w->delta, o, hd)); MGF_TRY(append(ctx, w->bpk, 4 * o, pack_records(c0, hd, he, c1)));
+  MGF_TRY(append(ctx, w->tb_c, o, tc));
   MGF_TRY(append(ctx, w->tb_r, o, tr)); MGF_TRY(append(ctx, w->fb_c, o, fc)); MGF_TRY(append(ctx, w->fb_r, o, fr));
   MGF_TRY(append(ctx, w->pcount, o, hp));
   MGF_TRY(append(ctx, w->lp0, kMaxParts * o, l0)); MGF_TRY(append(ctx, w->lp1, kMaxParts * o, l1));
@@ -987,7 +985,7 @@
   const size_t slot = w->permuted ? w->h_slot_of[r->index] : (size_t)r->index;
   float4 s[4], e, d;
   MGF_TRY(d2h(w->ctx, s, w->srec.p + 4 * slot, 4));
-  MGF_TRY(d2h(w->ctx, &e, w->einfo.p + slot, 1));
+  MGF_TRY(d2h(w->ctx, &e, w->bpk.p + 4 * slot + 2, 1));
   MGF_TRY(d2h(w->ctx, &d, w->delta.p + slot, 1));
   if (vel) { vel->linear = {s[0].x, s[0].y, s[0].z}; vel->angular = {s[0].w, s[1].x, s[1].y}; }
   if (info) {
diff --git a/mgf_amd/csrc/k_bodies.h b/mgf_amd/csrc/k_bodies.h
--- a/mgf_amd/csrc/k_bodies.h
+++ b/mgf_amd/csrc/k_bodies.h
@@ -16,6 +16,12 @@
 __device__ __forceinline__ float4 mk4(V3 v, float w) { return make_float4(v.x, v.y, v.z, w); }
 __device__ __forceinline__ float u2f(uint32_t u) { return __builtin_bit_cast(float, u); }
 __device__ __forceinline__ uint32_t f2u(float f) { return __builtin_bit_cast(uint32_t, f); }
+
+template <int K>
+struct PackField {
+  float4* pk;
+  __device__ __forceinline__ float4& operator[](size_t i) const { return pk[4 * i + K]; }
+};
 
 struct Bodies {
   float4* x;
@@ -26,10 +32,10 @@
   float4* ctor;
   float4* imb;
   float4* delta;
-  float4* einfo;
-  float4* col0;
-  float4* col1;
   float4* bpk;
+  PackField<2> einfo;
+  PackField<0> col0;
+  PackField<3> col1;
   float4* tb_c;
   float4* tb_r;
   float4* fb_c;
@@ -161,9 +167,6 @@
       s_rec[wv][2 * 65 + lane] = make_float4(I.c[0].y, I.c[0].z, I.c[1].x, I.c[1].y);
       s_rec[wv][3 * 65 + lane] = make_float4(I.c[1].z, I.c[2].x, I.c[2].y, I.c[2].z);
       B.delta[i] = mk4(d, p1.w);
-      B.einfo[i] = mk4(x + d, p0.w);
-      B.col0[i] = mk4(col.p, col.r);
-      B.col1[i] = mk4(col.d, u2f((uint32_t)col.kind));
       s_rec[wv][4 * 65 + lane] = mk4(col.p, col.r); s_rec[wv][5 * 65 + lane] = mk4(d, p1.w);
       s_rec[wv][6 * 65 + lane] = mk4(x + d, p0.w); s_rec[wv][7 * 65 + lane] = mk4(col.d, u2f((uint32_t)col.kind));
       B.tb_c[i] = mk4(tb.c, 0.0f);
@@ -203,7 +206,7 @@
       const int f = it * 64 + lane, rec = f >> 2, k = f & 3;
       if (i0 + (uint32_t)rec < n) {
         B.srec[4 * (size_t)i0 + f] = s_rec[wv][k * 65 + rec];
-        if (B.bpk) B.bpk[4 * (size_t)i0 + f] = s_rec[wv][(4 + k) * 65 + rec];
+        B.bpk[4 * (size_t)i0 + f] = s_rec[wv][(4 + k) * 65 + rec];
       }
     }
   }
@@ -251,6 +254,10 @@
   }
 }
 
+__global__ __launch_bounds__(kBlock) void k_pack_motion(Bodies B, uint32_t n) {
+  uint32_t i = blockIdx.x * kBlock + threadIdx.x;
+  if (i < n) B.bpk[4 * (size_t)i + 1] = B.delta[i];
+}
 __global__ __launch_bounds__(kBlock) void k_refresh_einfo(Bodies B, uint32_t n) {
   uint32_t i = blockIdx.x * kBlock + threadIdx.x;
   if (i < n) B.einfo[i] = mk4(xyz(B.x[i]) + xyz(B.delta[i]), B.einfo[i].w);
diff --git a/mgf_amd/csrc/k_broadphase.h b/mgf_amd/csrc/k_broadphase.h
--- a/mgf_amd/csrc/k_broadphase.h
+++ b/mgf_amd/csrc/k_broadphase.h
@@ -385,7 +385,7 @@
 }
 
 __device__ __forceinline__ void scatter_leaf(uint32_t body, const Lbvh& T, const float4* fb_c, const float4* fb_r, const uint32_t* cell_of,
-                                             const uint32_t* rank, uint32_t* brank, const float4* col0, const float4* delta, const float4* tb_c,
+                                             const uint32_t* rank, uint32_t* brank, PackField<0> col0, const float4* delta, const float4* tb_c,
                                              const float4* tb_r, const SceneBounds* sb, float pad_abs, float min_frac, const SceneBounds* box = nullptr,
                                              float3 wide_limit = make_float3(0.0f, 0.0f, 0.0f), uint32_t n_owned = 0u) {
   if (body >= T.n) return;
@@ -407,7 +407,7 @@
   brank[body] = p;
 }
 __global__ __launch_bounds__(kBlock) void k_scatter_leaves(Lbvh T, const float4* fb_c, const float4* fb_r, const uint32_t* cell_of,
-                                                           const uint32_t* rank, uint32_t* brank, const float4* col0, const float4* delta, const float4* tb_c,
+                                                           const uint32_t* rank, uint32_t* brank, PackField<0> col0, const float4* delta, const float4* tb_c,
                                                            const float4* tb_r, const SceneBounds* sb, float pad_abs, float min_frac, const SceneBounds* box = nullptr,
                                                            float3 wide_limit = make_float3(0.0f, 0.0f, 0.0f), uint32_t n_owned = 0u) {
   scatter_leaf(blockIdx.x * kBlock + threadIdx.x, T, fb_c, fb_r, cell_of, rank, brank, col0, delta, tb_c, tb_r, sb, pad_abs, min_frac, box, wide_limit, n_owned);
@@ -784,9 +784,7 @@
   return k;
 }
 __device__ __forceinline__ Comp load_comp_moving(const Bodies& B, uint32_t i, V3* v) {
-  float4 c0, c1, dl;
-  if (B.bpk) { c0 = B.bpk[4 * (size_t)i]; dl = B.bpk[4 * (size_t)i + 1]; c1 = B.bpk[4 * (size_t)i + 3]; }
-  else { c0 = B.col0[i]; c1 = B.col1[i]; dl = B.delta[i]; }
+  const float4 c0 = B.bpk[4 * (size_t)i], dl = B.bpk[4 * (size_t)i + 1], c1 = B.bpk[4 * (size_t)i + 3];
   Comp k; k.p = xyz(c0); k.r = c0.w; k.d = xyz(c1); k.kind = (int)f2u(c1.w);
   *v = xyz(dl);
   return k;
diff --git a/mgf_amd/csrc/k_contacts.h b/mgf_amd/csrc/k_contacts.h
--- a/mgf_amd/csrc/k_contacts.h
+++ b/mgf_amd/csrc/k_contacts.h
@@ -656,9 +656,9 @@
 
 struct BodyPack { float4 c0, dl, ei; };
 __device__ __forceinline__ BodyPack load_pack(const Bodies& B, uint32_t i, bool with_collider) {
+  (void)with_collider;
   BodyPack P;
-  if (B.bpk) { P.c0 = B.bpk[4 * i]; P.dl = B.bpk[4 * i + 1]; P.ei = B.bpk[4 * i + 2]; }
-  else { P.c0 = with_collider ? B.col0[i] : make_float4(0, 0, 0, 0); P.dl = B.delta[i]; P.ei = B.einfo[i]; }
+  P.c0 = B.bpk[4 * (size_t)i]; P.dl = B.bpk[4 * (size_t)i + 1]; P.ei = B.bpk[4 * (size_t)i + 2];
   return P;
 }
 
@@ -780,7 +780,7 @@
   NContact* t_out;
   uint32_t *tcn, *tpos;
   const uint32_t* guard;
-  const float4* col1;
+  PackField<3> col1;
   const uint32_t* pcount; const float4 *wp0, *wp1;
   uint32_t check; uint32_t* flag;
 };
@@ -939,7 +939,7 @@
 __global__ __launch_bounds__(kBlock) void k_terrain_contacts(TerrainContacts A) { terrain_contacts_job<GEN>(A, blockIdx.x, gridDim.x); }
 template <int GEN>
 __global__ __launch_bounds__(kBlock) void k_scatter_leaves_tc(Lbvh T, const float4* fb_c, const float4* fb_r, const uint32_t* cell_of,
-                                                              const uint32_t* rank, uint32_t* brank, const float4* col0, const float4* delta, const float4* tb_c,
+                                                              const uint32_t* rank, uint32_t* brank, PackField<0> col0, const float4* delta, const float4* tb_c,
                                                               const float4* tb_r, const SceneBounds* sb, float pad_abs, float min_frac, TerrainContacts A, uint32_t tc_blocks,
                                                               const SceneBounds* box, float3 wide_limit, uint32_t n_owned) {
   if (blockIdx.x < tc_blocks) { terrain_contacts_job<GEN>(A, blockIdx.x, tc_blocks); return; }
@@ -998,7 +998,7 @@
 template <bool SPH>
 __device__ __forceinline__ Comp pack_comp(const Bodies& B, uint32_t i, const BodyPack& P) {
   Comp X; X.p = xyz(P.c0); X.r = P.c0.w; X.d = mk3(0.0f, 0.0f, 0.0f); X.kind = KIND_SPHERE;
-  if (!SPH) { const float4 c1 = B.bpk ? B.bpk[4 * (size_t)i + 3] : B.col1[i]; X.d = xyz(c1); X.kind = (int)f2u(c1.w); }
+  if (!SPH) { const float4 c1 = B.col1[i]; X.d = xyz(c1); X.kind = (int)f2u(c1.w); }
   return X;
 }
 template <bool SPH>
diff --git a/mgf_amd/csrc/k_tiles.h b/mgf_amd/csrc/k_tiles.h
--- a/mgf_amd/csrc/k_tiles.h
+++ b/mgf_amd/csrc/k_tiles.h
@@ -157,11 +157,8 @@
   B.srec[4 * i + 2] = make_float4(o[26], o[27], o[28], o[29]);
   B.srec[4 * i + 3] = make_float4(o[30], o[31], o[32], o[33]);
   B.delta[i] = mk4(d, o[35]);
-  B.einfo[i] = mk4(x + d, o[34]);
   Comp k; k.kind = (int)f2u(o[16]); k.p = mk3(o[17], o[18], o[19]); k.d = mk3(o[20], o[21], o[22]); k.r = o[23];
-  B.col0[i] = mk4(k.p, k.r);
-  B.col1[i] = mk4(k.d, o[16]);
-  if (B.bpk) { B.bpk[4 * i] = mk4(k.p, k.r); B.bpk[4 * i + 1] = mk4(d, o[35]); B.bpk[4 * i + 2] = mk4(x + d, o[34]); B.bpk[4 * i + 3] = mk4(k.d, o[16]); }
+  B.bpk[4 * i] = mk4(k.p, k.r); B.bpk[4 * i + 1] = mk4(d, o[35]); B.bpk[4 * i + 2] = mk4(x + d, o[34]); B.bpk[4 * i + 3] = mk4(k.d, o[16]);
   Box tb = swept_bounds(k, d);
   const bool parts_in = rec > (uint32_t)kGhostFloatsPlain;
   const uint32_t pc = parts_in ? min(f2u(o[36]), (uint32_t)kTileParts) : 0u;
@@ -270,9 +267,9 @@
     case 8: return B.ctor + i;
     case 9: case 10: case 11: return B.imb + 3 * (size_t)i + (e - 9);
     case 12: return B.delta + i;
-    case 13: return B.einfo + i;
-    case 14: return B.col0 + i;
-    case 15: return B.col1 + i;
+    case 13: return &B.einfo[i];
+    case 14: return &B.col0[i];
+    case 15: return &B.col1[i];
     case 16: return B.tb_c + i;
     case 17: return B.tb_r + i;
     case 18: return B.fb_c + i;
@@ -467,7 +464,7 @@
   slot_of[e] = k;
 }
 
-__global__ __launch_bounds__(kBlock) void k_kind_mask(const float4* col1, const uint32_t* pcount, uint32_t base, uint32_t m, uint32_t* mask) {
+__global__ __launch_bounds__(kBlock) void k_kind_mask(PackField<3> col1, const uint32_t* pcount, uint32_t base, uint32_t m, uint32_t* mask) {
   uint32_t t = blockIdx.x * kBlock + threadIdx.x;
   if (t >= m) return;
   const uint32_t pc = pcount ? pcount[base + t] : 0u;
diff --git a/mgf_amd/csrc/mgf_hip.hip b/mgf_amd/csrc/mgf_hip.hip
--- a/mgf_amd/csrc/mgf_hip.hip
+++ b/mgf_amd/csrc/mgf_hip.hip
@@ -119,6 +119,12 @@
   MGF_TRY(buf.ensure(old_n + add.size(), ctx->stream, true, old_n));
   return h2d(ctx, buf.p + old_n, add.data(), add.size());
 }
+static std::vector<float4> pack_records(const std::vector<float4>& c0, const std::vector<float4>& dl, const std::vector<float4>& ei,
+                                        const std::vector<float4>& c1) {
+  std::vector<float4> r(4 * c0.size());
+  for (size_t i = 0; i < c0.size(); ++i) { r[4 * i] = c0[i]; r[4 * i + 1] = dl[i]; r[4 * i + 2] = ei[i]; r[4 * i + 3] = c1[i]; }
+  return r;
+}
 
 extern "C" mgf_status mgf_exclusive_scan_u32(mgf_ctx* ctx, const uint32_t* in, int64_t n, uint32_t* out) {
   MGF_TRY(ctx_bind(ctx));
```
